# ooowedyn/InkLayer

Measured on AMD Instinct MI355X. Metric: sketches/sec end-to-end (GroundingDINO+SAM) at 1024x1024, higher is better.
Workload: dtype f16 (MFMA, f32 accumulate; f32 residual/norm/softmax; split-f16 = fp32-grade operands for patch-embed, neck, mask decoder)

## Files before the change

### include/inklayer_hip.h

```cpp
#ifndef INKLAYER_HIP_H
#define INKLAYER_HIP_H

#include <stdint.h>

#ifdef __cplusplus
extern "C" {
#endif

#define INK_ABI_VERSION 8
int ink_abi_version(void);

typedef struct InkGemm {
  const void* A;
  const void* W;
  const float* bias;
  const float* col_scale;
  const float* residual;
  const int32_t* row_map;
  void* C;
  int32_t M, N, K;
  int32_t lda, ldw, ldr, ldc;
  int32_t act;
  int32_t c_f16;
} InkGemm;
#define INK_ACT_NONE 0
#define INK_ACT_GELU 1
#define INK_ACT_RELU 2
int ink_gemm_f16(const InkGemm* p, void* stream);
int ink_gemm_set_variant(int32_t v);
int ink_gemm_query_variant(int32_t M, int32_t N, int32_t K);

int ink_layernorm_rows(const float* x, int64_t ldx, const float* gamma, const float* beta,
                       float eps, const int32_t* gather, int32_t rows_out, int32_t C,
                       void* out_f16, float* out_f32, int64_t ldo, int32_t act, int32_t split,
                       const float* add, int64_t ld_add, const int32_t* add_batch_rows, int32_t rows_per_batch,
                       void* stream);

int ink_add_cvt_f16(const float* a, const float* b, int64_t n_b, void* out_f16, int64_t n,
                    void* stream);
int ink_add_split_f16(const float* a, const float* b, int64_t n_b, void* out_f16, int64_t n, int32_t C,
                      void* stream);
int ink_add_f32(const float* a, const float* b, int64_t n_b, float* out, int64_t n, void* stream);

typedef struct InkAttn {
  const void* Q; const void* K; const void* V;
  void* O;
  int64_t ldq, ldk, ldv, ldo;
  int32_t n_batch, n_heads, n_q, n_k, head_dim;
  float scale;
  int32_t bias_mode;
  int32_t grid_w;
  const int32_t* q_batch_rows;
  const int32_t* kv_batch_rows;
  const float* rel_h; const float* rel_w;
  const void* rel_aug;
  const float* dense_bias; const float* dense_mask;
  int32_t n_mask; int32_t rel_f16;
  const int32_t* tok_rows;
  const void* pad_k; const void* pad_v;
} InkAttn;
int ink_flash_attn(const InkAttn* p, void* stream);

int ink_relpos_bias64_f16(const void* Q, int64_t ldq, const float* rel_pos_h, const float* rel_pos_w, int32_t n_batch,
                          int32_t n_heads, int32_t head_dim, float scale, void* out_h_f16, void* out_w_f16, void* stream);

int ink_relpos_bias(const void* Q, int64_t ldq, const float* rel_pos_h, const float* rel_pos_w,
                    int32_t S, int32_t n_batch, int32_t n_heads, int32_t head_dim, float scale,
                    const int32_t* tok_rows, float* out_h, float* out_w, void* out_aug_f16,
                    void* stream);

int ink_sam_patchify(const void* image_u8, int32_t h, int32_t w, int32_t L, int32_t P,
                     const float* mean3, const float* std3, int32_t chan_reverse, int32_t split,
                     void* out_f16, void* stream);

int ink_resize_bilinear_u8(const void* src_u8, int32_t h, int32_t w, void* dst_u8, int32_t oh, int32_t ow,
                           const int32_t* xbounds, const int32_t* xcoef, int32_t kx,
                           const int32_t* ybounds, const int32_t* ycoef, int32_t ky, void* tmp_u8,
                           void* stream);

int ink_im2col3x3_f16(const void* in_f16, int32_t B, int32_t H, int32_t W, int32_t C, void* out_f16,
                      void* stream);

int ink_sam_pe_encode(const float* coords01, const float* gauss, int32_t N, int32_t F,
                      const float* add, int32_t n_add, float* out, void* stream);

int ink_sam_prompt_tokens(const float* points, const int32_t* labels, int32_t n_pts, int32_t pad, const float* boxes,
                          const float* gauss, int32_t F, const float* point_emb, const float* not_a_point,
                          const float* out_tok, float input_size, int32_t P, float* out, void* stream);

int ink_sam_mask_embed(const float* mask, const float* emb, const int32_t* emb_rows, const float* params,
                       int32_t n_params, float eps, int32_t P, int32_t g, float* keys, void* split_f16, void* stream);

int ink_sam_mask_logits(const float* up, const float* hyper, int32_t n, int32_t g, int32_t C,
                        float* out, void* stream);

int ink_sam_postprocess(const float* low, int32_t n, int32_t S, int32_t L, int32_t in_h,
                        int32_t in_w, int32_t out_h, int32_t out_w, float thr, void* out_u8,
                        float* out_logits, void* stream);

int ink_ms_deform_attn_forward(const float* value, const int64_t* spatial_shapes_host,
                               const int64_t* level_start_index_host, const float* sampling_loc,
                               const float* attn_weight, int32_t B, int32_t S, int32_t M, int32_t C,
                               int32_t Q, int32_t L, int32_t P, int32_t im2col_step, float* out,
                               void* stream);

int ink_ms_deform_attn_forward_dev(const void* value, const int64_t* spatial_shapes,
                                   const int64_t* level_start_index, const void* sampling_loc,
                                   const void* attn_weight, int32_t dtype, int32_t B, int32_t S, int32_t M,
                                   int32_t C, int32_t Q, int32_t L, int32_t P, int32_t im2col_step,
                                   void* out, void* stream);
int ink_ms_deform_attn_backward_dev(const void* value, const int64_t* spatial_shapes,
                                    const int64_t* level_start_index, const void* sampling_loc,
                                    const void* attn_weight, const void* grad_output, int32_t dtype,
                                    int32_t B, int32_t S, int32_t M, int32_t C, int32_t Q, int32_t L,
                                    int32_t P, int32_t im2col_step, void* grad_value,
                                    void* grad_sampling_loc, void* grad_attn_weight, void* stream);

int ink_msda_fused(const void* value_f16, const float* proj, int64_t ldp, const float* ref,
                   int32_t ref_dim, int64_t ref_q_stride, int64_t ref_b_stride,
                   const int32_t* shapes_host, int32_t B, int32_t S, int32_t Q, void* out_f16,
                   void* stream);

int ink_swin_patchify(const void* image_u8, int32_t h, int32_t w, const float* mean3,
                      const float* std3, void* out_f16, void* stream);

int ink_layernorm_merge4(const float* x, int64_t ldx, const float* gamma, const float* beta, float eps,
                         const int32_t* gather4, int32_t rows, int32_t C, void* out_f16, void* stream);

int ink_groupnorm_nhwc(const float* x, int32_t B, int32_t T, int32_t C, int32_t G, const float* gamma,
                       const float* beta, float eps, float* stats_ws, float* out,
                       int64_t out_batch_stride, void* stream);

int ink_gather_rows(const float* x, int64_t ldx, int64_t x_batch_rows, const int32_t* idx,
                    int64_t idx_batch_stride, int32_t rows_per_batch, int32_t B, int32_t C,
                    void* out_f16, float* out_f32, void* stream);

int ink_biattn_fusion(const void* QV_f16, const void* KL_f16, int32_t B, int32_t S, int32_t T, int32_t E,
                      float scale, float* scores_ws, float* stats_ws, float* partial_ws, int32_t chunk,
                      void* out_v_f16, void* out_l_f16, void* stream);

int ink_attn_fewkeys(const void* Q, int64_t ldq, const void* K, int64_t ldk, const void* V, int64_t ldv,
                     int32_t B, int32_t n_q, int32_t n_k, int32_t n_heads, int32_t head_dim, float scale,
                     const uint8_t* blocked, const int32_t* q_batch_rows, const float* q_add, int32_t io_f32, void* O,
                     int64_t ldo, void* stream);

int ink_attn_fewq(const void* Q, int64_t ldq, const void* K, int64_t ldk, const void* V, int64_t ldv,
                  int32_t n_batch, int32_t n_q, int32_t n_k, int32_t n_heads, int32_t head_dim, float scale,
                  const int32_t* q_batch_rows, const int32_t* kv_batch_rows, const float* k_add, void* O, int64_t ldo,
                  void* stream);

int ink_biattn_colstats(const float* scores, int32_t B, int32_t S, int32_t HT, float* part_ws, float* stats, void* stream);

int ink_fusion_fold_workspace(int32_t B, int32_t S, int64_t* out_floats);
int ink_fusion_fold(float* v_f32, int32_t B, int32_t S, const float* lnv_g, const float* lnv_b, float eps,
                    const float* text_k_f32, const float* text_vl_f32, int64_t ld_text, int32_t T, const void* Wq_f16,
                    const float* bq, const void* Wvv_f16, const float* bvv, const void* Wo_f16, const float* bo,
                    const float* gamma_v, float scale, float* ws, void* out_l_f16, const float* pos, void* out16_pos,
                    void* out16, void* stream);

int ink_sam_upscale_pack(const void* ws_f16, void* blob_f16, void* stream);
int ink_sam_upscale_tail(const float* u0, int64_t ld_tok, int32_t n, int32_t g, const float* ln_g, const float* ln_b, float eps,
                         const void* blob_f16, const float* b3, const float* hyper, int32_t n_masks, float* low,
                         void* stream);

int ink_proj256_ln_pack(const void* ws_f16, void* blob_f16, void* stream);
int ink_proj256_ln(const float* a_f32, const void* blob_f16, const float* bias, const float* res_f32,
                   const int32_t* res_batch_rows, int32_t rows_per_batch, const float* ln_g, const float* ln_b, float eps,
                   int64_t rows, float* out_f32, void* out_split_f16, void* stream);

int ink_ffn256_pack_bytes(int32_t hid, int32_t with_pre, int64_t* out_bytes);
int ink_ffn256_pack(const void* w1_f16, const float* b1, const void* w2_f16, int32_t hid, const void* wpre_f16, void* blob,
                    void* stream);
int ink_ffn256_fused(const void* x_f16, int64_t ldx, const float* res_f32, const void* blob, const float* b2,
                     const float* ln_g, const float* ln_b, float eps, int32_t M, int32_t hid, const float* pre_bias,
                     const float* pre_ln_g, const float* pre_ln_b, float* out_f32, void* stream);

int ink_topk_rowmax(const float* logits, int32_t B, int32_t S, int32_t T, int32_t K, int32_t* out_idx,
                    float* out_val, void* cand_ws, void* stream);

int ink_sine_embed4(const float* ref, const float* dim_t, int32_t N, void* out_f16, void* stream);

int ink_box_refine(const float* delta, int64_t ldd, const float* ref, int32_t N, int32_t ref_is_logit,
                   float* out, void* stream);

int ink_mask_cleanup_workspace_ints(int32_t n, int32_t H, int32_t W, int32_t k, int64_t* out_ints);
int ink_mask_cleanup(const void* masks_u8, int32_t n, int32_t H, int32_t W, int32_t k, int32_t area_threshold,
                     double aspect_threshold, void* tmp_a_u8, void* tmp_b_u8, int32_t* workspace, void* out_u8,
                     void* stream);

int ink_mask_sketch_iou_counts(const void* masks_u8, const void* sketch_rgb_u8, int32_t n, int32_t H, int32_t W,
                               void* bits_ws_u64, int32_t* counts, void* stream);

int ink_sam_amg_stats(const float* low, int32_t n, const int32_t* index, int32_t m, const int32_t* m_dev, int32_t S,
                      int32_t L, int32_t in_h, int32_t in_w, int32_t crop_h, int32_t crop_w, double thr, double offset,
                      int32_t x0, int32_t y0, int32_t orig_h, int32_t orig_w, int32_t* table, void* planes_u64,
                      float* out_logits, void* stream);

int ink_mask_rle_counts(const void* planes_u64, const int32_t* select, int32_t k, int32_t H, int32_t W,
                        int32_t* n_counts, void* stream);
int ink_mask_rle_write(const void* planes_u64, const int32_t* select, int32_t k, int32_t H, int32_t W,
                       const int32_t* offsets, int32_t* counts, void* stream);

int ink_mask_small_regions_workspace_ints(int32_t k, int32_t H, int32_t W, int64_t* out_ints);
int ink_mask_small_regions(const void* planes_u64, int32_t k, int32_t H, int32_t W, int32_t min_area, int32_t holes,
                           void* tmp_planes_u64, int32_t* workspace, void* out_planes_u64, int32_t* changed, void* stream);

int ink_box_nms(const float* boxes, const float* scores, int32_t n, float iou_threshold, void* workspace_u64,
                int32_t* keep, int32_t* n_keep, void* stream);

int ink_refine_sketch_planes(const void* rgb_u8, int32_t H, int32_t W, void* planes4_u64, int32_t* max_ws, void* stream);

int ink_bitplane_pack(const void* img_u8, int32_t n, int32_t H, int32_t W, int32_t thresh, void* planes_u64, void* stream);

int ink_refine_depth_samples(const void* mask_planes, int32_t n, const float* depth, const int32_t* pts_yx, int32_t P,
                             int32_t H, int32_t W, float* vals, void* inside_u8, void* stream);

int ink_refine_pair_tables(const void* mask_planes, const void* sketch_planes4, int32_t n, int32_t H, int32_t W,
                           const int32_t* rect, void* dil_ws_planes, int32_t* pair, int32_t* per_mask,
                           int32_t* sketch_area, void* stream);

int ink_refine_composite(const void* mask_planes, const int32_t* order, int32_t n_ranks, int32_t H, int32_t W,
                         void* label_u8, int32_t* hist256, void* stream);

int ink_refine_relabel_clean(const void* label_u8, const void* map256_u8, int32_t H, int32_t W, void* out_label_u8,
                             void* stream);

int ink_refine_grow_workspace(int32_t H, int32_t W, int64_t* plane_words, int64_t* cc_ints);
int ink_refine_grow(const void* label_u8, const void* sketch_planes4, int32_t H, int32_t W, void* planes_ws,
                    int32_t* cc_ws, int32_t* flags256, void* out_label_u8, int32_t* bbox256x4, int32_t* unl_yx,
                    int32_t unl_cap, int32_t* unl_count, void* stream);

int ink_refine_query_dists(const void* label_u8, const int32_t* q_yx, const void* cand256_bits, int32_t Q, int32_t H,
                           int32_t W, int32_t* d2_Qx256, void* stream);

int ink_refine_finalize(void* label_u8, const int32_t* assign_yxl, int32_t A, const void* sketch_planes4, int32_t H,
                        int32_t W, void* planes_ws3, void* extra_plane, int32_t* extra_count, void* stream);

int ink_host_sparse_sample(const uint8_t* rgb_u8, int32_t H, int32_t W, int32_t* out_yx, int32_t cap, int32_t* count);
int ink_host_assign_unlabeled(const int32_t* q_yx, int32_t Q, const int32_t* boxes, int32_t nb, const int32_t* box2mask,
                              const int32_t* d2, const uint8_t* nonempty, int32_t n_masks, int32_t* out_label);

int ink_depth_patchify(const void* image_u8, int32_t H, int32_t W, int32_t nh, int32_t nw, int32_t P, int32_t KP,
                       const double* mean3, const double* std3, int32_t chan_reverse, void* out_f16, void* stream);

int ink_resize_bilinear_ac_nhwc(const float* in, int32_t B, int32_t h, int32_t w, int32_t C, int32_t H, int32_t W,
                                float* out_f32, void* out_f16, void* stream);

int ink_im2col3x3_ex_f16(const void* in_f16, int32_t B, int32_t H, int32_t W, int32_t C, int32_t stride, int32_t relu,
                         void* out_f16, void* stream);

int ink_layers_otsu_planes(const void* gray_u8, int32_t n, int32_t H, int32_t W, int32_t invert, int32_t* hist,
                           int32_t* thresh, void* out_planes, void* stream);

int ink_layers_dilate(const void* planes, int32_t n, int32_t H, int32_t W, int32_t kernel_size, int32_t iterations,
                      void* tmp_planes, void* out_planes, void* stream);

int ink_layers_border_band(const void* planes, int32_t n, int32_t H, int32_t W, int32_t band, int32_t* flags,
                           void* stream);

int ink_layers_components_workspace_ints(int32_t n, int32_t H, int32_t W, int64_t* out_ints);
int ink_layers_components(const void* planes, int32_t n, int32_t H, int32_t W, int32_t mode, void* tmp_planes3,
                          int32_t* workspace, void* out_planes, void* stream);

int ink_layers_chamfer_workspace_ints(int32_t n, int32_t H, int32_t W, int64_t* out_ints);
int ink_layers_chamfer(const void* mask_planes, const void* stroke_planes, int32_t n, int32_t H, int32_t W,
                       int32_t safety_margin, int32_t full, int32_t* dist, int32_t* workspace, int32_t* min_out,
                       int32_t* shrink_out, void* out_planes, void* stream);

int ink_layers_mask_tables(const void* masks_u8, int32_t n, int32_t H, int32_t W, int32_t* bbox, int32_t* overlap,
                           void* stream);

int ink_layers_assemble(const void* sketch_rgb_u8, const void* masks_u8, const void* bg_planes, const int32_t* bbox,
                        const int32_t* overlap, int32_t n, int32_t H, int32_t W, void* sketch_layers_u8,
                        void* edit_masks_u8, void* debug_u8, void* stream);

int ink_layers_composite(const void* inpainted_rgb_u8, const void* sketch_layer_u8, int32_t H, int32_t W,
                         void* out_rgb_u8, void* stream);

int ink_layers_gray(const void* rgb_u8, int32_t n, int32_t H, int32_t W, void* gray_u8, void* stream);

int ink_layers_rgba(const void* gray_u8, const void* bg_planes, int32_t n, int32_t H, int32_t W, void* rgba_u8,
                    void* stream);


int ink_inp_contrast(const void* rgb_u8, int32_t H, int32_t W, float factor, void* sum_u64, void* out_rgb_u8,
                     void* stream);

int ink_inp_bilateral(const void* rgb_u8, int32_t H, int32_t W, const float* tables, void* out_rgb_u8, void* stream);

int ink_inp_mask_prepare(const void* mask_u8, int32_t H, int32_t W, int32_t dilate_iterations, int32_t blur,
                         void* tmp2_u8, void* out_u8, void* stream);

int ink_inp_resize_u8(const void* src_u8, int32_t h, int32_t w, int32_t channels, void* dst_u8, int32_t oh, int32_t ow,
                      const int32_t* xbounds, const int32_t* xcoef, int32_t kx, const int32_t* ybounds,
                      const int32_t* ycoef, int32_t ky, void* tmp_u8, void* stream);

int ink_inp_condition(const void* rgb_u8, const void* mask_u8, int32_t H, int32_t W, float* out_f32, void* stream);
// ... 19 lines not shown
```

### inklayer_amd/_lib.py

```python
from __future__ import annotations

import ctypes as C
import os
from pathlib import Path

_LIB_PATH = Path(__file__).resolve().parent / "lib" / "libinklayer_hip.so"
_lib = None

c_void_p, c_int, c_i64, c_float = C.c_void_p, C.c_int32, C.c_int64, C.c_float


class InkGemm(C.Structure):
    _fields_ = [
        ("A", c_void_p), ("W", c_void_p), ("bias", c_void_p), ("col_scale", c_void_p),
        ("residual", c_void_p), ("row_map", c_void_p), ("C", c_void_p),
        ("M", c_int), ("N", c_int), ("K", c_int),
        ("lda", c_int), ("ldw", c_int), ("ldr", c_int), ("ldc", c_int),
        ("act", c_int), ("c_f16", c_int),
    ]


class InkAttn(C.Structure):
    _fields_ = [
        ("Q", c_void_p), ("K", c_void_p), ("V", c_void_p), ("O", c_void_p),
        ("ldq", c_i64), ("ldk", c_i64), ("ldv", c_i64), ("ldo", c_i64),
        ("n_batch", c_int), ("n_heads", c_int), ("n_q", c_int), ("n_k", c_int),
        ("head_dim", c_int), ("scale", c_float), ("bias_mode", c_int), ("grid_w", c_int),
        ("q_batch_rows", c_void_p), ("kv_batch_rows", c_void_p),
        ("rel_h", c_void_p), ("rel_w", c_void_p), ("rel_aug", c_void_p),
        ("dense_bias", c_void_p), ("dense_mask", c_void_p), ("n_mask", c_int), ("rel_f16", c_int),
        ("tok_rows", c_void_p), ("pad_k", c_void_p), ("pad_v", c_void_p),
    ]


SIGNATURES = {
    "ink_abi_version": [],
    "ink_gemm_f16": [C.POINTER(InkGemm), c_void_p],
    "ink_gemm_set_variant": [c_int],
    "ink_gemm_query_variant": [c_int, c_int, c_int],
    "ink_layernorm_rows": [c_void_p, c_i64, c_void_p, c_void_p, c_float, c_void_p, c_int, c_int,
                           c_void_p, c_void_p, c_i64, c_int, c_int, c_void_p, c_i64, c_void_p, c_int, c_void_p],
    "ink_add_split_f16": [c_void_p, c_void_p, c_i64, c_void_p, c_i64, c_int, c_void_p],
    "ink_add_cvt_f16": [c_void_p, c_void_p, c_i64, c_void_p, c_i64, c_void_p],
    "ink_add_f32": [c_void_p, c_void_p, c_i64, c_void_p, c_i64, c_void_p],
    "ink_flash_attn": [C.POINTER(InkAttn), c_void_p],
    "ink_sam_patchify": [c_void_p, c_int, c_int, c_int, c_int, C.POINTER(c_float), C.POINTER(c_float),
                         c_int, c_int, c_void_p, c_void_p],
    "ink_im2col3x3_f16": [c_void_p, c_int, c_int, c_int, c_int, c_void_p, c_void_p],
    "ink_resize_bilinear_u8": [c_void_p, c_int, c_int, c_void_p, c_int, c_int, c_void_p, c_void_p, c_int,
                               c_void_p, c_void_p, c_int, c_void_p, c_void_p],
    "ink_sam_pe_encode": [c_void_p, c_void_p, c_int, c_int, c_void_p, c_int, c_void_p, c_void_p],
    "ink_sam_mask_logits": [c_void_p, c_void_p, c_int, c_int, c_int, c_void_p, c_void_p],
    "ink_sam_prompt_tokens": [c_void_p, c_void_p, c_int, c_int, c_void_p, c_void_p, c_int, c_void_p, c_void_p,
                              c_void_p, c_float, c_int, c_void_p, c_void_p],
    "ink_sam_mask_embed": [c_void_p, c_void_p, c_void_p, c_void_p, c_int, c_float, c_int, c_int, c_void_p, c_void_p,
                           c_void_p],
    "ink_sam_postprocess": [c_void_p, c_int, c_int, c_int, c_int, c_int, c_int, c_int, c_float,
                            c_void_p, c_void_p, c_void_p],
    "ink_sam_amg_stats": [c_void_p, c_int, c_void_p, c_int, c_void_p, c_int, c_int, c_int, c_int, c_int, c_int, C.c_double,
                          C.c_double, c_int, c_int, c_int, c_int, c_void_p, c_void_p, c_void_p, c_void_p],
    "ink_mask_rle_counts": [c_void_p, c_void_p, c_int, c_int, c_int, c_void_p, c_void_p],
    "ink_mask_rle_write": [c_void_p, c_void_p, c_int, c_int, c_int, c_void_p, c_void_p, c_void_p],
    "ink_mask_small_regions_workspace_ints": [c_int, c_int, c_int, C.POINTER(c_i64)],
    "ink_mask_small_regions": [c_void_p, c_int, c_int, c_int, c_int, c_int, c_void_p, c_void_p, c_void_p, c_void_p,
                               c_void_p],
    "ink_box_nms": [c_void_p, c_void_p, c_int, c_float, c_void_p, c_void_p, c_void_p, c_void_p],
    "ink_ms_deform_attn_forward": [c_void_p, C.POINTER(c_i64), C.POINTER(c_i64), c_void_p, c_void_p, c_int,
                                   c_int, c_int, c_int, c_int, c_int, c_int, c_int, c_void_p, c_void_p],
    "ink_ms_deform_attn_forward_dev": [c_void_p, c_void_p, c_void_p, c_void_p, c_void_p, c_int, c_int, c_int, c_int,
                                       c_int, c_int, c_int, c_int, c_int, c_void_p, c_void_p],
    "ink_ms_deform_attn_backward_dev": [c_void_p, c_void_p, c_void_p, c_void_p, c_void_p, c_void_p, c_int, c_int, c_int,
                                        c_int, c_int, c_int, c_int, c_int, c_int, c_void_p, c_void_p, c_void_p,
                                        c_void_p],
    "ink_msda_fused": [c_void_p, c_void_p, c_i64, c_void_p, c_int, c_i64, c_i64, C.POINTER(c_int), c_int,
                       c_int, c_int, c_void_p, c_void_p],
    "ink_swin_patchify": [c_void_p, c_int, c_int, C.POINTER(c_float), C.POINTER(c_float), c_void_p, c_void_p],
    "ink_layernorm_merge4": [c_void_p, c_i64, c_void_p, c_void_p, c_float, c_void_p, c_int, c_int, c_void_p,
                             c_void_p],
    "ink_groupnorm_nhwc": [c_void_p, c_int, c_int, c_int, c_int, c_void_p, c_void_p, c_float, c_void_p,
                           c_void_p, c_i64, c_void_p],
    "ink_gather_rows": [c_void_p, c_i64, c_i64, c_void_p, c_i64, c_int, c_int, c_int, c_void_p, c_void_p,
                        c_void_p],
    "ink_biattn_fusion": [c_void_p, c_void_p, c_int, c_int, c_int, c_int, c_float, c_void_p, c_void_p,
                          c_void_p, c_int, c_void_p, c_void_p, c_void_p],
    "ink_biattn_colstats": [c_void_p, c_int, c_int, c_int, c_void_p, c_void_p, c_void_p],
    "ink_fusion_fold_workspace": [c_int, c_int, C.POINTER(c_i64)],
    "ink_relpos_bias64_f16": [c_void_p, c_i64, c_void_p, c_void_p, c_int, c_int, c_int, c_float, c_void_p, c_void_p, c_void_p],
    "ink_proj256_ln_pack": [c_void_p, c_void_p, c_void_p],
    "ink_proj256_ln": [c_void_p, c_void_p, c_void_p, c_void_p, c_void_p, c_int, c_void_p, c_void_p, c_float, c_i64, c_void_p,
                       c_void_p, c_void_p],
    "ink_sam_upscale_pack": [c_void_p, c_void_p, c_void_p],
    "ink_sam_upscale_tail": [c_void_p, c_i64, c_int, c_int, c_void_p, c_void_p, c_float, c_void_p, c_void_p, c_void_p,
                             c_int, c_void_p, c_void_p],
    "ink_ffn256_pack_bytes": [c_int, c_int, C.POINTER(c_i64)],
    "ink_ffn256_pack": [c_void_p, c_void_p, c_void_p, c_int, c_void_p, c_void_p, c_void_p],
    "ink_ffn256_fused": [c_void_p, c_i64, c_void_p, c_void_p, c_void_p, c_void_p, c_void_p, c_float, c_int, c_int,
                         c_void_p, c_void_p, c_void_p, c_void_p, c_void_p],
    "ink_fusion_fold": [c_void_p, c_int, c_int, c_void_p, c_void_p, c_float, c_void_p, c_void_p, c_i64, c_int, c_void_p,
                        c_void_p, c_void_p, c_void_p, c_void_p, c_void_p, c_void_p, c_float, c_void_p, c_void_p, c_void_p,
                        c_void_p, c_void_p, c_void_p],
    "ink_attn_fewkeys": [c_void_p, c_i64, c_void_p, c_i64, c_void_p, c_i64, c_int, c_int, c_int, c_int, c_int,
                         c_float, c_void_p, c_void_p, c_void_p, c_int, c_void_p, c_i64, c_void_p],
    "ink_attn_fewq": [c_void_p, c_i64, c_void_p, c_i64, c_void_p, c_i64, c_int, c_int, c_int, c_int, c_int,
                      c_float, c_void_p, c_void_p, c_void_p, c_void_p, c_i64, c_void_p],
    "ink_topk_rowmax": [c_void_p, c_int, c_int, c_int, c_int, c_void_p, c_void_p, c_void_p, c_void_p],
    "ink_sine_embed4": [c_void_p, c_void_p, c_int, c_void_p, c_void_p],
    "ink_box_refine": [c_void_p, c_i64, c_void_p, c_int, c_int, c_void_p, c_void_p],
    "ink_mask_cleanup_workspace_ints": [c_int, c_int, c_int, c_int, C.POINTER(c_i64)],
    "ink_mask_cleanup": [c_void_p, c_int, c_int, c_int, c_int, c_int, C.c_double, c_void_p, c_void_p, c_void_p,
                         c_void_p, c_void_p],
    "ink_mask_sketch_iou_counts": [c_void_p, c_void_p, c_int, c_int, c_int, c_void_p, c_void_p, c_void_p],
    "ink_refine_sketch_planes": [c_void_p, c_int, c_int, c_void_p, c_void_p, c_void_p],
    "ink_bitplane_pack": [c_void_p, c_int, c_int, c_int, c_int, c_void_p, c_void_p],
    "ink_refine_depth_samples": [c_void_p, c_int, c_void_p, c_void_p, c_int, c_int, c_int, c_void_p, c_void_p, c_void_p],
    "ink_refine_pair_tables": [c_void_p, c_void_p, c_int, c_int, c_int, c_void_p, c_void_p, c_void_p, c_void_p,
                               c_void_p, c_void_p],
    "ink_refine_composite": [c_void_p, c_void_p, c_int, c_int, c_int, c_void_p, c_void_p, c_void_p],
    "ink_refine_relabel_clean": [c_void_p, c_void_p, c_int, c_int, c_void_p, c_void_p],
    "ink_refine_grow_workspace": [c_int, c_int, C.POINTER(c_i64), C.POINTER(c_i64)],
    "ink_refine_grow": [c_void_p, c_void_p, c_int, c_int, c_void_p, c_void_p, c_void_p, c_void_p, c_void_p, c_void_p,
                        c_int, c_void_p, c_void_p],
    "ink_refine_query_dists": [c_void_p, c_void_p, c_void_p, c_int, c_int, c_int, c_void_p, c_void_p],
    "ink_refine_finalize": [c_void_p, c_void_p, c_int, c_void_p, c_int, c_int, c_void_p, c_void_p, c_void_p, c_void_p],
    "ink_host_sparse_sample": [c_void_p, c_int, c_int, c_void_p, c_int, c_void_p],
    "ink_host_assign_unlabeled": [c_void_p, c_int, c_void_p, c_int, c_void_p, c_void_p, c_void_p, c_int, c_void_p],
    "ink_depth_patchify": [c_void_p, c_int, c_int, c_int, c_int, c_int, c_int, C.POINTER(C.c_double), C.POINTER(C.c_double),
                           c_int, c_void_p, c_void_p],
    "ink_resize_bilinear_ac_nhwc": [c_void_p, c_int, c_int, c_int, c_int, c_int, c_int, c_void_p, c_void_p, c_void_p],
    "ink_im2col3x3_ex_f16": [c_void_p, c_int, c_int, c_int, c_int, c_int, c_int, c_void_p, c_void_p],
    "ink_layers_otsu_planes": [c_void_p, c_int, c_int, c_int, c_int, c_void_p, c_void_p, c_void_p, c_void_p],
    "ink_layers_dilate": [c_void_p, c_int, c_int, c_int, c_int, c_int, c_void_p, c_void_p, c_void_p],
    "ink_layers_border_band": [c_void_p, c_int, c_int, c_int, c_int, c_void_p, c_void_p],
    "ink_layers_components_workspace_ints": [c_int, c_int, c_int, C.POINTER(c_i64)],
    "ink_layers_components": [c_void_p, c_int, c_int, c_int, c_int, c_void_p, c_void_p, c_void_p, c_void_p],
    "ink_layers_chamfer_workspace_ints": [c_int, c_int, c_int, C.POINTER(c_i64)],
    "ink_layers_chamfer": [c_void_p, c_void_p, c_int, c_int, c_int, c_int, c_int, c_void_p, c_void_p, c_void_p, c_void_p,
                           c_void_p, c_void_p],
    "ink_layers_mask_tables": [c_void_p, c_int, c_int, c_int, c_void_p, c_void_p, c_void_p],
    "ink_layers_assemble": [c_void_p, c_void_p, c_void_p, c_void_p, c_void_p, c_int, c_int, c_int, c_void_p, c_void_p,
                            c_void_p, c_void_p],
    "ink_layers_composite": [c_void_p, c_void_p, c_int, c_int, c_void_p, c_void_p],
    "ink_layers_gray": [c_void_p, c_int, c_int, c_int, c_void_p, c_void_p],
    "ink_layers_rgba": [c_void_p, c_void_p, c_int, c_int, c_int, c_void_p, c_void_p],
    "ink_inp_contrast": [c_void_p, c_int, c_int, c_float, c_void_p, c_void_p, c_void_p],
    "ink_inp_bilateral": [c_void_p, c_int, c_int, c_void_p, c_void_p, c_void_p],
    "ink_inp_mask_prepare": [c_void_p, c_int, c_int, c_int, c_int, c_void_p, c_void_p, c_void_p],
    "ink_inp_resize_u8": [c_void_p, c_int, c_int, c_int, c_void_p, c_int, c_int, c_void_p, c_void_p, c_int,
                          c_void_p, c_void_p, c_int, c_void_p, c_void_p],
    "ink_inp_condition": [c_void_p, c_void_p, c_int, c_int, c_void_p, c_void_p],
    "ink_inp_cleanup": [c_void_p, c_int, c_int, c_void_p, c_void_p, c_void_p, c_void_p, c_void_p],
    "ink_inp_soft_blend": [c_void_p, c_void_p, c_void_p, c_int, c_int, c_void_p, c_void_p, c_void_p, c_void_p],
    "ink_inp_luma": [c_void_p, c_int, c_int, c_int, c_void_p, c_void_p],
    "ink_inp_unsharp": [c_void_p, c_int, c_int, c_int, C.c_uint32, C.c_uint32, c_int, c_int, c_void_p, c_void_p, c_void_p],
    "ink_inp_rgba_cut": [c_void_p, c_void_p, c_int, c_int, c_void_p, c_void_p],
    "ink_relpos_bias": [c_void_p, c_i64, c_void_p, c_void_p, c_int, c_int, c_int, c_int, c_float,
                        c_void_p, c_void_p, c_void_p, c_void_p, c_void_p],
}


class InkLayerHipError(RuntimeError):
    pass


def lib_path() -> Path:
    return Path(os.environ.get("INKLAYER_HIP_LIB", _LIB_PATH))


def lib() -> C.CDLL:
    global _lib
    if _lib is None:
        p = lib_path()
        if not p.exists():
            raise InkLayerHipError(
                f"{p} not found: build it with `python -m inklayer_amd.build` "
                "(there is no CPU/eager fallback for the InkLayer hot path)")
        try:
            import torch
        except ImportError:
            pass
        l = C.CDLL(str(p))
        for name, argtypes in SIGNATURES.items():
            fn = getattr(l, name)
            fn.argtypes = argtypes
            fn.restype = C.c_int
        _lib = l
    return _lib


def check(rc: int, what: str) -> None:
    if rc != 0:
        raise InkLayerHipError(f"{what} failed: " + {1: "bad argument", 2: "HIP launch error"}.get(rc, str(rc)))
```

### inklayer_amd/csrc/attn_few.hip

```cpp
#include "common.h"
#include "../../include/inklayer_hip.h"

namespace {

__device__ __forceinline__ void load8(const f16* p, float* d) {
  const f16x8 v = *(const f16x8*)p;
#pragma unroll
  for (int j = 0; j < 8; ++j) d[j] = (float)v[j];
}
__device__ __forceinline__ void load8(const float* p, float* d) {
  const f32x4 a = *(const f32x4*)p, b = *(const f32x4*)(p + 4);
#pragma unroll
  for (int j = 0; j < 4; ++j) { d[j] = a[j]; d[4 + j] = b[j]; }
}
__device__ __forceinline__ void store8(f16* p, const float* d) {
  f16x8 v;
#pragma unroll
  for (int j = 0; j < 8; ++j) v[j] = (f16)d[j];
  *(f16x8*)p = v;
}
__device__ __forceinline__ void store8(float* p, const float* d) {
  *(f32x4*)p = (f32x4){d[0], d[1], d[2], d[3]};
  *(f32x4*)(p + 4) = (f32x4){d[4], d[5], d[6], d[7]};
}

template <int HD, typename T>
__global__ __launch_bounds__(256) void attn_fewkeys_kernel(const T* __restrict__ Q, int64_t ldq,
                                                           const T* __restrict__ K, int64_t ldk,
                                                           const T* __restrict__ V, int64_t ldv, int B,
                                                           int n_q, int n_k, int n_heads, float scale,
                                                           const uint8_t* __restrict__ blocked,
                                                           const int32_t* __restrict__ q_rows,
                                                           const float* __restrict__ q_add,
                                                           T* __restrict__ O, int64_t ldo) {
  const int64_t gid = (int64_t)blockIdx.x * 256 + threadIdx.x;
  if (gid >= (int64_t)B * n_q * n_heads) return;
  const int h = (int)(gid % n_heads);
  const int64_t bq = gid / n_heads;
  const int b = (int)(bq / n_q), q = (int)(bq % n_q);
  float qv[HD];
  const T* qp = Q + (q_rows ? (int64_t)q_rows[b] + q : bq) * ldq + h * HD;
#pragma unroll
  for (int i = 0; i < HD / 8; ++i) load8(qp + 8 * i, qv + 8 * i);
  if (q_add) {
    const float* ap = q_add + ((int64_t)q * n_heads + h) * HD;
#pragma unroll
    for (int i = 0; i < HD; ++i) qv[i] += ap[i];
  }
  float sc[16];
  float mx = -3.0e38f;
  for (int t = 0; t < n_k; ++t) {
    const T* kp = K + ((int64_t)b * n_k + t) * ldk + h * HD;
    float d = 0.f;
#pragma unroll
    for (int i = 0; i < HD / 8; ++i) {
      float kv[8];
      load8(kp + 8 * i, kv);
#pragma unroll
      for (int j = 0; j < 8; ++j) d = fmaf(qv[8 * i + j], kv[j], d);
    }
    d *= scale;
    if (blocked && blocked[q * n_k + t]) d = -3.0e38f;
    sc[t] = d;
    mx = fmaxf(mx, d);
  }
  float sum = 0.f;
  for (int t = 0; t < n_k; ++t) { sc[t] = sc[t] <= -1.0e38f ? 0.f : expf(sc[t] - mx); sum += sc[t]; }
  const float inv = 1.f / sum;
  float acc[HD];
#pragma unroll
  for (int i = 0; i < HD; ++i) acc[i] = 0.f;
  for (int t = 0; t < n_k; ++t) {
    const T* vp = V + ((int64_t)b * n_k + t) * ldv + h * HD;
    const float pw = sc[t] * inv;
#pragma unroll
    for (int i = 0; i < HD / 8; ++i) {
      float vv[8];
      load8(vp + 8 * i, vv);
#pragma unroll
      for (int j = 0; j < 8; ++j) acc[8 * i + j] = fmaf(pw, vv[j], acc[8 * i + j]);
    }
  }
  T* op = O + bq * ldo + h * HD;
#pragma unroll
  for (int i = 0; i < HD / 8; ++i) store8(op + 8 * i, acc + 8 * i);
}


template <int NK>
__global__ __launch_bounds__(256) void attn_fewkeys16_f32_kernel(const float* __restrict__ Q, int64_t ldq,
                                                                 const float* __restrict__ K, int64_t ldk,
                                                                 const float* __restrict__ V, int64_t ldv, int B,
                                                                 int n_q, int n_heads, float scale,
                                                                 const int32_t* __restrict__ q_rows,
                                                                 const float* __restrict__ q_add,
                                                                 float* __restrict__ O, int64_t ldo) {
  const int64_t gid = (int64_t)blockIdx.x * 256 + threadIdx.x;
  if (gid >= (int64_t)B * n_q * n_heads * 4) return;
  const int part = (int)(gid & 3);
  const int h = (int)((gid >> 2) % n_heads);
  const int64_t bq = (gid >> 2) / n_heads;
  const int b = (int)(bq / n_q), q = (int)(bq % n_q);
  const int col = h * 16 + 4 * part;
  f32x4 qv = *(const f32x4*)(Q + (q_rows ? (int64_t)q_rows[b] + q : bq) * ldq + col);
  if (q_add) qv += *(const f32x4*)(q_add + (int64_t)q * n_heads * 16 + col);
  qv *= scale * 1.44269504088896340736f;
  const float* kp = K + (int64_t)b * NK * ldk + col;
  const float* vp = V + (int64_t)b * NK * ldv + col;
  f32x4 kv[NK], vv[NK];
#pragma unroll
  for (int t = 0; t < NK; ++t) {
    kv[t] = *(const f32x4*)(kp + (int64_t)t * ldk);
    vv[t] = *(const f32x4*)(vp + (int64_t)t * ldv);
  }
  float sc[NK];
  float mx = -3.0e38f;
#pragma unroll
  for (int t = 0; t < NK; ++t) {
    float d = (qv[0] * kv[t][0] + qv[1] * kv[t][1]) + (qv[2] * kv[t][2] + qv[3] * kv[t][3]);
    d += __builtin_bit_cast(float, __builtin_amdgcn_update_dpp(0, __builtin_bit_cast(int, d), 0xB1, 0xF, 0xF, false));
    d += __builtin_bit_cast(float, __builtin_amdgcn_update_dpp(0, __builtin_bit_cast(int, d), 0x4E, 0xF, 0xF, false));
    sc[t] = d;
    mx = fmaxf(mx, d);
  }
  float sum = 0.f;
#pragma unroll
  for (int t = 0; t < NK; ++t) { sc[t] = __builtin_amdgcn_exp2f(sc[t] - mx); sum += sc[t]; }
  const float inv = 1.f / sum;
  f32x4 acc = {0.f, 0.f, 0.f, 0.f};
#pragma unroll
  for (int t = 0; t < NK; ++t) acc += (sc[t] * inv) * vv[t];
  *(f32x4*)(O + bq * ldo + col) = acc;
}

template <int QW>
__global__ __launch_bounds__(512) void attn_fewq16_kernel(const float* __restrict__ Q, int64_t ldq,
                                                          const float* __restrict__ K, int64_t ldk,
                                                          const float* __restrict__ V, int64_t ldv, int n_q,
                                                          int n_k, int n_heads, float scale,
                                                          const int32_t* __restrict__ q_rows,
                                                          const int32_t* __restrict__ kv_rows,
                                                          const float* __restrict__ k_add,
                                                          float* __restrict__ O, int64_t ldo) {
  constexpr int KSPLIT = 2, HD = 16, HB = 4, TK = 64;
  constexpr int ROWE = HB * HD;
  constexpr int CH = 4, NCH = ROWE / CH;
  constexpr int NU = TK * NCH / 256;
  constexpr bool Q_IN_LDS = QW > 2;
  extern __shared__ __attribute__((aligned(16))) char fewq_smem[];
  const int grp = threadIdx.x >> 8;
  float* sk = (float*)fewq_smem + grp * 2 * TK * ROWE;
  float* sv = sk + TK * ROWE;
  const int hgroups = n_heads / HB;
  const int b = blockIdx.x / hgroups, h0 = (blockIdx.x % hgroups) * HB;
  const int tid = threadIdx.x & 255, lane = tid & 63, wave = tid >> 6;
  const int per = ((n_k + KSPLIT - 1) / KSPLIT + TK - 1) / TK * TK;
  const int k_lo = grp * per, k_hi = min(n_k, k_lo + per);
  const int kl = lane >> 2, hl = lane & 3;
  const int64_t q0 = q_rows ? (int64_t)q_rows[b] : (int64_t)b * n_q;
  const int64_t k0 = kv_rows ? (int64_t)kv_rows[b] : (int64_t)b * n_k;
  float* sq = (float*)fewq_smem + KSPLIT * 2 * TK * ROWE;
  float qr[QW][HD];
  if (!Q_IN_LDS || (grp == 0 && kl == 0)) {
    const float sc2 = scale * 1.44269504088896340736f;
#pragma unroll
    for (int j = 0; j < QW; ++j) {
      const int qi = QW * wave + j;
      const float* pq = Q + (q0 + (qi < n_q ? qi : 0)) * ldq + (h0 + hl) * HD;
      load8(pq, qr[j]);
      load8(pq + 8, qr[j] + 8);
#pragma unroll
      for (int e = 0; e < HD; ++e) qr[j][e] *= sc2;
      if constexpr (Q_IN_LDS) {
        store8(sq + (qi * HB + hl) * HD, qr[j]);
        store8(sq + (qi * HB + hl) * HD + 8, qr[j] + 8);
      }
    }
  }
  float m[QW], l[QW], acc[QW][HD];
#pragma unroll
  for (int j = 0; j < QW; ++j) {
    m[j] = -3.0e38f;
    l[j] = 0.f;
#pragma unroll
    for (int i = 0; i < HD; ++i) acc[j][i] = 0.f;
  }
  f32x4 rk[NU], rv[NU];
  auto fetch = [&](int t0) {
#pragma unroll
    for (int u = 0; u < NU; ++u) {
      const int c = tid + 256 * u, row = c / NCH, col = c % NCH;
      rk[u] = rv[u] = (f32x4){0.f, 0.f, 0.f, 0.f};
      if (t0 + row < k_hi) {
        rk[u] = *(const f32x4*)(K + (k0 + t0 + row) * ldk + h0 * HD + col * CH);
        rv[u] = *(const f32x4*)(V + (k0 + t0 + row) * ldv + h0 * HD + col * CH);
        if (k_add) rk[u] += *(const f32x4*)(k_add + (int64_t)(t0 + row) * n_heads * HD + h0 * HD + col * CH);
      }
    }
  };
  fetch(k_lo);
  for (int t0 = k_lo; t0 < k_lo + per; t0 += TK) {
    __syncthreads();
#pragma unroll
    for (int u = 0; u < NU; ++u) {
      const int c = tid + 256 * u, row = c / NCH, col = c % NCH;
      *(f32x4*)(sk + row * ROWE + col * CH) = rk[u];
      *(f32x4*)(sv + row * ROWE + col * CH) = rv[u];
    }
    __syncthreads();
    if (t0 + TK < k_hi) fetch(t0 + TK);
    float d[QW][TK / 16];
#pragma unroll
    for (int kk = 0; kk < TK / 16; ++kk) {
      const int key = kk * 16 + kl;
      float kf[HD];
      load8(sk + key * ROWE + hl * HD, kf);
      load8(sk + key * ROWE + hl * HD + 8, kf + 8);
      const bool in = t0 + key < k_hi;
#pragma unroll
      for (int j = 0; j < QW; ++j) {
        float qf[HD];
        if constexpr (Q_IN_LDS) {
          load8(sq + ((QW * wave + j) * HB + hl) * HD, qf);
          load8(sq + ((QW * wave + j) * HB + hl) * HD + 8, qf + 8);
        } else {
#pragma unroll
          for (int e = 0; e < HD; ++e) qf[e] = qr[j][e];
        }
        float a0 = 0.f;
#pragma unroll
        for (int e = 0; e < 8; ++e) {
          a0 = fmaf(qf[e], kf[e], a0);
          a0 = fmaf(qf[8 + e], kf[8 + e], a0);
        }
        d[j][kk] = in ? a0 : -3.0e38f;
      }
    }
    float n[QW];
#pragma unroll
    for (int j = 0; j < QW; ++j) {
      n[j] = m[j];
#pragma unroll
      for (int kk = 0; kk < TK / 16; ++kk) n[j] = fmaxf(n[j], d[j][kk]);
      const float sj = __builtin_amdgcn_exp2f(m[j] - n[j]);
      l[j] *= sj;
#pragma unroll
      for (int e = 0; e < HD; ++e) acc[j][e] *= sj;
      m[j] = n[j];
    }
#pragma unroll
    for (int kk = 0; kk < TK / 16; ++kk) {
      const int key = kk * 16 + kl;
      float vf[HD];
      load8(sv + key * ROWE + hl * HD, vf);
      load8(sv + key * ROWE + hl * HD + 8, vf + 8);
      const bool in = t0 + key < k_hi;
#pragma unroll
      for (int j = 0; j < QW; ++j) {
        const float pj = in ? __builtin_amdgcn_exp2f(d[j][kk] - n[j]) : 0.f;
        l[j] += pj;
#pragma unroll
        for (int e = 0; e < HD; ++e) acc[j][e] = fmaf(pj, vf[e], acc[j][e]);
      }
    }
  }
#pragma unroll
  for (int j = 0; j < QW; ++j) {
#pragma unroll
    for (int o = 4; o < 64; o <<= 1) {
      const float mo = __shfl_xor(m[j], o, 64), lo = __shfl_xor(l[j], o, 64);
      const float mn = fmaxf(m[j], mo);
      const float a = __builtin_amdgcn_exp2f(m[j] - mn), bsc = __builtin_amdgcn_exp2f(mo - mn);
      l[j] = l[j] * a + lo * bsc;
#pragma unroll
      for (int i = 0; i < HD; ++i) acc[j][i] = acc[j][i] * a + __shfl_xor(acc[j][i], o, 64) * bsc;
      m[j] = mn;
    }
  }
  __syncthreads();
  float* st = (float*)fewq_smem;
  if (grp > 0 && kl == 0) {
#pragma unroll
    for (int j = 0; j < QW; ++j) {
      float* ps = st + ((((grp - 1) * 4 + wave) * QW + j) * 4 + hl) * 18;
      ps[0] = m[j];
      ps[1] = l[j];
#pragma unroll
      for (int i = 0; i < HD; ++i) ps[2 + i] = acc[j][i];
    }
  }
  __syncthreads();
  if (grp > 0) return;
  if (kl == 0) {
#pragma unroll
    for (int g2 = 1; g2 < KSPLIT; ++g2)
#pragma unroll
      for (int j = 0; j < QW; ++j) {
        const float* ps = st + ((((g2 - 1) * 4 + wave) * QW + j) * 4 + hl) * 18;
        const float mo = ps[0], mn = fmaxf(m[j], mo);
        const float a = __builtin_amdgcn_exp2f(m[j] - mn), bsc = __builtin_amdgcn_exp2f(mo - mn);
        l[j] = l[j] * a + ps[1] * bsc;
#pragma unroll
        for (int i = 0; i < HD; ++i) acc[j][i] = acc[j][i] * a + ps[2 + i] * bsc;
        m[j] = mn;
      }
#pragma unroll
    for (int j = 0; j < QW; ++j) {
      const int qi = QW * wave + j;
      if (qi < n_q) {
        const float inv = 1.f / l[j];
#pragma unroll
        for (int i = 0; i < HD; ++i) acc[j][i] *= inv;
        float* op = O + ((int64_t)b * n_q + qi) * ldo + (h0 + hl) * HD;
        store8(op, acc[j]);
        store8(op + 8, acc[j] + 8);
      }
    }
  }
}

}

extern "C" int ink_attn_fewkeys(const void* Q, int64_t ldq, const void* K, int64_t ldk, const void* V,
                                int64_t ldv, int32_t B, int32_t n_q, int32_t n_k, int32_t n_heads,
                                int32_t head_dim, float scale, const uint8_t* blocked,
                                const int32_t* q_batch_rows, const float* q_add, int32_t io_f32, void* O,
                                int64_t ldo, void* stream) {
  INK_CHECK_ARG(Q && K && V && O && B > 0 && n_q > 0 && n_k > 0 && n_k <= 16 && n_heads > 0);
  INK_CHECK_ARG(ldq % 8 == 0 && ldk % 8 == 0 && ldv % 8 == 0 && ldo % 8 == 0);
  INK_CHECK_ARG(io_f32 == 0 || io_f32 == 1);
  INK_CHECK_ARG((((uintptr_t)Q | (uintptr_t)K | (uintptr_t)V | (uintptr_t)O) & 15) == 0);
  INK_CHECK_ARG(!q_add || (((uintptr_t)q_add & 15) == 0));
  const int64_t total = (int64_t)B * n_q * n_heads;
  const dim3 grid((unsigned)((total + 255) / 256)), block(256);
  hipStream_t s = (hipStream_t)stream;
#define INK_FEWKEYS(HD, T)                                                                                     \
  hipLaunchKernelGGL((attn_fewkeys_kernel<HD, T>), grid, block, 0, s, (const T*)Q, ldq, (const T*)K, ldk,      \
                     (const T*)V, ldv, B, n_q, n_k, n_heads, scale, blocked, q_batch_rows, q_add, (T*)O, ldo)
  if (head_dim == 32 && !io_f32) INK_FEWKEYS(32, f16);
  else if (head_dim == 64 && !io_f32) INK_FEWKEYS(64, f16);
  else if (!io_f32) return INK_ERR_ARG;
  else if (head_dim == 32) INK_FEWKEYS(32, float);
  else if (head_dim == 16 && !blocked && n_k >= 7) {
    const dim3 g4((unsigned)((total * 4 + 255) / 256));
#define INK_FEWKEYS16(NK)                                                                                        \
  case NK:                                                                                                      \
    hipLaunchKernelGGL(attn_fewkeys16_f32_kernel<NK>, g4, block, 0, s, (const float*)Q, ldq, (const float*)K, ldk, \
                       (const float*)V, ldv, B, n_q, n_heads, scale, q_batch_rows, q_add, (float*)O, ldo);         \
    break
    switch (n_k) {
      INK_FEWKEYS16(7); INK_FEWKEYS16(8); INK_FEWKEYS16(9); INK_FEWKEYS16(10); INK_FEWKEYS16(11);
      INK_FEWKEYS16(12); INK_FEWKEYS16(13); INK_FEWKEYS16(14); INK_FEWKEYS16(15); INK_FEWKEYS16(16);
      default: return INK_ERR_ARG;
    }
#undef INK_FEWKEYS16
  } else if (head_dim == 16) INK_FEWKEYS(16, float);
  else return INK_ERR_ARG;
#undef INK_FEWKEYS
  return ink_launch_status();
}

extern "C" int ink_attn_fewq(const void* Q, int64_t ldq, const void* K, int64_t ldk, const void* V, int64_t ldv,
                             int32_t n_batch, int32_t n_q, int32_t n_k, int32_t n_heads, int32_t head_dim,
                             float scale, const int32_t* q_batch_rows, const int32_t* kv_batch_rows,
                             const float* k_add, void* O, int64_t ldo, void* stream) {
  INK_CHECK_ARG(Q && K && V && O && n_batch > 0 && n_q > 0 && n_q <= 16 && n_k > 0 && n_heads > 0);
  INK_CHECK_ARG(head_dim == 16 && n_heads % 4 == 0);
  INK_CHECK_ARG(ldq % 8 == 0 && ldk % 8 == 0 && ldv % 8 == 0 && ldo % 8 == 0);
  INK_CHECK_ARG((((uintptr_t)Q | (uintptr_t)K | (uintptr_t)V | (uintptr_t)O) & 15) == 0);
  INK_CHECK_ARG(!k_add || ((uintptr_t)k_add & 15) == 0);
  constexpr int lds2 = 2 * 2 * 64 * 64 * 4, lds4 = lds2 + 16 * 64 * 4;
  static bool attr = ((void)hipFuncSetAttribute((const void*)attn_fewq16_kernel<2>,
                                                hipFuncAttributeMaxDynamicSharedMemorySize, lds2),
                      (void)hipFuncSetAttribute((const void*)attn_fewq16_kernel<4>,
                                                hipFuncAttributeMaxDynamicSharedMemorySize, lds4), true);
  (void)attr;
  const bool wide = n_q > 8;
  hipLaunchKernelGGL(wide ? attn_fewq16_kernel<4> : attn_fewq16_kernel<2>, dim3(n_batch * (n_heads / 4)), dim3(512),
                     wide ? lds4 : lds2, (hipStream_t)stream, (const float*)Q, ldq, (const float*)K, ldk,
                     (const float*)V, ldv, n_q, n_k, n_heads, scale, q_batch_rows, kv_batch_rows, k_add, (float*)O, ldo);
  return ink_launch_status();
}
```

### inklayer_amd/csrc/common.h

```cpp
#pragma once
#include <hip/hip_runtime.h>
#include <stdint.h>

typedef _Float16 f16;
typedef _Float16 f16x2 __attribute__((ext_vector_type(2)));
typedef _Float16 f16x4 __attribute__((ext_vector_type(4)));
typedef _Float16 f16x8 __attribute__((ext_vector_type(8)));
typedef float f32x2 __attribute__((ext_vector_type(2)));
typedef float f32x4 __attribute__((ext_vector_type(4)));
typedef float f32x16 __attribute__((ext_vector_type(16)));
typedef short s16x4 __attribute__((ext_vector_type(4)));

#define INK_OK 0
#define INK_ERR_ARG 1
#define INK_ERR_LAUNCH 2

#define INK_CHECK_ARG(cond)            \
  do {                                 \
    if (!(cond)) return INK_ERR_ARG;   \
  } while (0)

static inline int ink_launch_status() {
  hipError_t e = hipGetLastError();
  return e == hipSuccess ? INK_OK : INK_ERR_LAUNCH;
}

__device__ __forceinline__ float wave_sum(float v) {
#pragma unroll
  for (int o = 32; o > 0; o >>= 1) v += __shfl_xor(v, o, 64);
  return v;
}
__device__ __forceinline__ float wave_max(float v) {
#pragma unroll
  for (int o = 32; o > 0; o >>= 1) v = fmaxf(v, __shfl_xor(v, o, 64));
  return v;
}

__device__ __forceinline__ float gelu_erf(float x) {
  const float u = fabsf(x) * 0.84932180028801904272f;
  const float t = __builtin_amdgcn_rcpf(fmaf(0.27273748087922250f, u, 1.0f));
  float pl = fmaf(1.061405429f, t, -1.453152027f);
  pl = fmaf(pl, t, 1.421413741f);
  pl = fmaf(pl, t, -0.284496736f);
  pl = fmaf(pl, t, 0.254829592f);
  const float e = pl * t * __builtin_amdgcn_exp2f(-(u * u));
  return fmaf(-0.5f * fabsf(x), e, fmaxf(x, 0.0f));
}

__device__ __forceinline__ int xcd_remap(int bid, int nwg) {
  const int q = nwg >> 3, r = nwg & 7, x = bid & 7;
  return (x < r ? x * (q + 1) : r * (q + 1) + (x - r) * q) + (bid >> 3);
}
```

### inklayer_amd/csrc/gemm.hip

```cpp
#include <stdlib.h>

#include "common.h"
#include "../../include/inklayer_hip.h"

namespace {

template <int BK> struct Swz;
template <> struct Swz<64> {
  static __device__ __forceinline__ int f(int row) { return row & 7; }
};
template <> struct Swz<32> {
  static __device__ __forceinline__ int f(int row) { return (-(row >> 2)) & 3; }
};

typedef __attribute__((address_space(1))) const void* gptr_t;
typedef __attribute__((address_space(3))) void* lptr_t;

__device__ __forceinline__ bool residual_preloaded(const InkGemm& p) {
  return p.residual && p.act == INK_ACT_NONE && !p.col_scale;
}

template <int TM>
__device__ __forceinline__ void wave_rows(int (&rows)[TM], const InkGemm& p, int mw, int lane) {
#pragma unroll
  for (int ti = 0; ti < TM; ++ti) {
    const int m = mw + ti * 16 + (lane & 15);
    int r = -1;
    if (m < p.M) r = p.row_map ? p.row_map[m] : m;
    rows[ti] = r;
  }
}

template <int TM, int TN>
__device__ __forceinline__ void init_wave_tile(f32x4 (&acc)[TM][TN], const InkGemm& p, const int (&rows)[TM], int nw,
                                               int lane) {
  const int fq = lane >> 4;
  const bool pre = residual_preloaded(p);
#pragma unroll
  for (int ti = 0; ti < TM; ++ti) {
    const int r = pre ? rows[ti] : -1;
    const float* rp = p.residual + (size_t)max(r, 0) * p.ldr + nw + fq * 4;
#pragma unroll
    for (int j = 0; j < TN; ++j) {
      acc[ti][j] = (f32x4){0.f, 0.f, 0.f, 0.f};
      if (r >= 0 && nw + j * 16 + fq * 4 < p.N) acc[ti][j] = *(const f32x4*)(rp + j * 16);
    }
  }
}

template <int TM, int TN>
__device__ __forceinline__ void add_bias_wave_tile(f32x4 (&acc)[TM][TN], const InkGemm& p, int nw, int lane) {
  const int fq = lane >> 4;
#pragma unroll
  for (int j = 0; j < TN; ++j) {
    const int n = nw + j * 16 + fq * 4;
    f32x4 bv = (f32x4){0.f, 0.f, 0.f, 0.f};
    if (p.bias && n < p.N) bv = *(const f32x4*)(p.bias + n);
#pragma unroll
    for (int ti = 0; ti < TM; ++ti) acc[ti][j] += bv;
  }
}

template <int TM, int TN, int OUT, int MODE = -1>
__device__ __forceinline__ void store_wave_tile(f32x4 (&acc)[TM][TN], const InkGemm& p, char* er,
                                                const int (&rows)[TM], int nw, int lane) {
  constexpr bool F16O = OUT == 1;
  constexpr int WNC = TN * 16, EP = WNC * 4 + 16;
  constexpr int ES = OUT == 0 ? 4 : 8;
  constexpr int CPRW = WNC / ES;
  constexpr int NIT = (16 * CPRW + 63) / 64;
  const int fr = lane & 15, fq = lane >> 4;
  const bool wide16 = OUT != 0 && (p.ldc % 8 == 0);
  const bool res_late = MODE < 0 && p.residual && !residual_preloaded(p);
  const int act = MODE < 0 ? p.act : MODE;
  const bool scaled = MODE < 0 && p.col_scale != nullptr;
  int row_of[NIT], n_of[NIT];
#pragma unroll
  for (int it = 0; it < NIT; ++it) {
    const int c = it * 64 + lane;
    row_of[it] = c < 16 * CPRW ? c / CPRW : 16;
    n_of[it] = nw + (c % CPRW) * ES;
  }

  add_bias_wave_tile<TM, TN>(acc, p, nw, lane);

#pragma unroll
  for (int ti = 0; ti < TM; ++ti) {
#pragma unroll
    for (int j = 0; j < TN; ++j) {
      f32x4 v = acc[ti][j];
      if (act == INK_ACT_GELU) {
#pragma unroll
        for (int r = 0; r < 4; ++r) v[r] = gelu_erf(v[r]);
      } else if (act == INK_ACT_RELU) {
#pragma unroll
        for (int r = 0; r < 4; ++r) v[r] = fmaxf(v[r], 0.f);
      }
      if (scaled) {
        const int n = nw + j * 16 + fq * 4;
        if (n < p.N) v *= *(const f32x4*)(p.col_scale + n);
      }
      if (F16O) {
        *(f16x4*)(er + fr * EP + (j * 16 + fq * 4) * 2) = (f16x4){(f16)v[0], (f16)v[1], (f16)v[2], (f16)v[3]};
      } else {
        *(f32x4*)(er + fr * EP + (j * 16 + fq * 4) * 4) = v;
      }
    }
#pragma unroll
    for (int it = 0; it < NIT; ++it) {
      int r = __builtin_amdgcn_ds_bpermute((row_of[it] & 15) << 2, rows[ti]);
      if (row_of[it] >= 16 || n_of[it] >= p.N) r = -1;
      if (r >= 0) {
        const int c_n = n_of[it];
        const char* src = er + row_of[it] * EP + (c_n - nw) * (F16O ? 2 : 4);
        if (F16O) {
          f16x8 d = *(const f16x8*)src;
          f16* dst = (f16*)p.C + (size_t)r * p.ldc + c_n;
          if (res_late) {
            const float* rp = p.residual + (size_t)r * p.ldr + c_n;
#pragma unroll
            for (int e = 0; e < 8; ++e)
              if (c_n + e < p.N) d[e] = (f16)((float)d[e] + rp[e]);
          }
          if (wide16 && c_n + 8 <= p.N) {
            *(f16x8*)dst = d;
          } else {
            *(f16x4*)dst = (f16x4){d[0], d[1], d[2], d[3]};
            if (c_n + 8 <= p.N) *(f16x4*)(dst + 4) = (f16x4){d[4], d[5], d[6], d[7]};
          }
        } else {
          f32x4 d = *(const f32x4*)src;
          if (res_late) d += *(const f32x4*)(p.residual + (size_t)r * p.ldr + c_n);
          *(f32x4*)((float*)p.C + (size_t)r * p.ldc + c_n) = d;
        }
      }
    }
  }
}

__device__ __forceinline__ void tile_of(int id, int ntm, int ntn, int group_m, int& mt, int& nt) {
  if (group_m > 1) {
    const int per = group_m * ntn;
    const int first = (id / per) * group_m;
    const int gsz = min(ntm - first, group_m);
    mt = first + (id % per) % gsz;
    nt = (id % per) / gsz;
  } else {
    mt = id / ntn;
    nt = id % ntn;
  }
}

constexpr int NS = 2;
template <int BM, int BN, int BK, int WM, int WN>
__global__ __launch_bounds__(WM * WN * 64) void gemm_f16_nt(InkGemm p, int group_m) {
  constexpr int NT = WM * WN * 64;
  constexpr int CPR = BK / 8;
  constexpr int ROWB = BK * 2;
  constexpr int TILE_A = BM * ROWB, TILE_W = BN * ROWB;
  constexpr int STAGE = TILE_A + TILE_W;
  constexpr int IT_A = (BM * CPR) / NT, IT_W = (BN * CPR) / NT;
  constexpr int TM = BM / WM / 16, TN = BN / WN / 16;
  static_assert((BM * CPR) % NT == 0 && (BN * CPR) % NT == 0, "tile/threads mismatch");
  extern __shared__ __attribute__((aligned(16))) char smem[];

  const int tid = threadIdx.x;
  const int lane = tid & 63;
  const int wave = tid >> 6;
  const int wm = wave / WN, wn = wave % WN;

  const int ntn = (p.N + BN - 1) / BN;
  const int ntm = (p.M + BM - 1) / BM;
  int mt, nt;
  tile_of(xcd_remap(blockIdx.x, ntm * ntn), ntm, ntn, group_m, mt, nt);
  const int m0 = mt * BM;
  const int n0 = nt * BN;

  const f16* __restrict__ A = (const f16*)p.A;
  const f16* __restrict__ W = (const f16*)p.W;

  const f16* srcA[IT_A];
  const f16* srcW[IT_W];
#pragma unroll
  for (int it = 0; it < IT_A; ++it) {
    const int pch = it * NT + tid;
    const int row = pch / CPR;
    const int lch = (pch % CPR) ^ Swz<BK>::f(row);
    srcA[it] = A + (size_t)min(m0 + row, p.M - 1) * p.lda + lch * 8;
  }
#pragma unroll
  for (int it = 0; it < IT_W; ++it) {
    const int pch = it * NT + tid;
    const int row = pch / CPR;
    const int lch = (pch % CPR) ^ Swz<BK>::f(row);
    srcW[it] = W + (size_t)min(n0 + row, p.N - 1) * p.ldw + lch * 8;
  }

  auto stage = [&](int buf, int kt) {
    char* base = smem + buf * STAGE;
#pragma unroll
    for (int it = 0; it < IT_A; ++it)
      __builtin_amdgcn_global_load_lds((gptr_t)(srcA[it] + kt * BK), (lptr_t)(base + (it * NT + wave * 64) * 16), 16, 0, 0);
#pragma unroll
    for (int it = 0; it < IT_W; ++it)
      __builtin_amdgcn_global_load_lds((gptr_t)(srcW[it] + kt * BK), (lptr_t)(base + TILE_A + (it * NT + wave * 64) * 16), 16, 0, 0);
  };

  int rows[TM];
  wave_rows<TM>(rows, p, m0 + wm * (BM / WM), lane);
  f32x4 acc[TM][TN];

  const int fr = lane & 15, fq = lane >> 4;
  const int offA = (wm * (BM / WM) + fr) * ROWB;
  const int offW = (wn * (BN / WN) + fr) * ROWB;
  const int swz = Swz<BK>::f(fr);

  const int nk = p.K / BK;
  auto compute = [&](int cur) {
    const char* bA = smem + cur * STAGE;
    const char* bW = bA + TILE_A;
#pragma unroll
    for (int kk = 0; kk < BK / 32; ++kk) {
      constexpr int AG = TM > 4 ? 4 : TM;
      f16x8 a[AG], w[TN];
      const int co = ((kk * 4 + fq) ^ swz) << 4;
#pragma unroll
      for (int j = 0; j < TN; ++j) w[j] = *(const f16x8*)(bW + offW + j * 16 * ROWB + co);
#pragma unroll
      for (int i0 = 0; i0 < TM; i0 += AG) {
#pragma unroll
        for (int i = 0; i < AG; ++i) a[i] = *(const f16x8*)(bA + offA + (i0 + i) * 16 * ROWB + co);
#pragma unroll
        for (int i = 0; i < AG; ++i)
#pragma unroll
          for (int j = 0; j < TN; ++j)
            acc[i0 + i][j] = __builtin_amdgcn_mfma_f32_16x16x32_f16(w[j], a[i], acc[i0 + i][j], 0, 0, 0);
      }
    }
  };

  stage(0, 0);
  init_wave_tile<TM, TN>(acc, p, rows, n0 + wn * (BN / WN), lane);
  for (int kt = 0; kt < nk; ++kt) {
    asm volatile("s_waitcnt vmcnt(0)" ::: "memory");
    __syncthreads();
    if (kt + 1 < nk) stage((kt + 1) & 1, kt + 1);
    compute(kt & 1);
  }

  constexpr int WNC = BN / WN;
  constexpr int EP = WNC * 4 + 16;
  static_assert(WM * WN * 16 * EP <= NS * STAGE, "epilogue patch must fit in the staging LDS");
  __syncthreads();
  char* er = smem + wave * (16 * EP);
  if (p.c_f16 == 1) {
    store_wave_tile<TM, TN, 1>(acc, p, er, rows, n0 + wn * WNC, lane);
  } else {
    store_wave_tile<TM, TN, 0>(acc, p, er, rows, n0 + wn * WNC, lane);
  }
}

constexpr int PP_RING = 4, PP_TN = 5;
__global__ __launch_bounds__(512) void gemm_f16_nt_pp(InkGemm p, int group_m) {
  constexpr int RING = PP_RING, TN = PP_TN;
  constexpr int BM = 256, BN = 64 * TN, BK = 32, NT = 512;
  constexpr int CPR = BK / 8, ROWB = BK * 2;
  constexpr int TILE_A = BM * ROWB, TILE_W = BN * ROWB, GRAN = TILE_A + TILE_W;
  constexpr int IT_A = (BM * CPR) / NT, IT_W = (BN * CPR) / NT;
  constexpr bool W_TAIL = (BN * CPR) % NT != 0;
  static_assert(!W_TAIL || (BN * CPR) % NT == NT / 2, "tail is exactly the first four waves");
  constexpr int LOADS = IT_A + IT_W;
  constexpr int TM = 8, WNC = 16 * TN;
  constexpr int AHEAD = RING - 2;
  constexpr int AG = 4;
  constexpr int EP = WNC * 4 + 16;
  static_assert(8 * 16 * EP <= RING * GRAN, "patch fits");
  extern __shared__ __attribute__((aligned(16))) char smem[];
  const int tid = threadIdx.x, lane = tid & 63;
  const int wave = __builtin_amdgcn_readfirstlane(tid >> 6);
  const int grp = wave >> 2, wn = wave & 3;
  const int fr = lane & 15, fq = lane >> 4;

  const int ntn = (p.N + BN - 1) / BN, ntm = (p.M + BM - 1) / BM;
  int mt, nt;
  tile_of(xcd_remap(blockIdx.x, ntm * ntn), ntm, ntn, group_m, mt, nt);
  const int m0 = mt * BM, n0 = nt * BN;
  const int G = p.K / BK;
  const f16* __restrict__ A = (const f16*)p.A;
  const f16* __restrict__ W = (const f16*)p.W;
  const f16* srcA[IT_A];
  const f16* srcW[IT_W + (W_TAIL ? 1 : 0)];
#pragma unroll
  for (int it = 0; it < IT_A; ++it) {
    const int pch = it * NT + tid, row = pch / CPR, lch = (pch % CPR) ^ Swz<BK>::f(row);
    srcA[it] = A + (size_t)min(m0 + row, p.M - 1) * p.lda + lch * 8;
  }
#pragma unroll
  for (int it = 0; it < IT_W + (W_TAIL ? 1 : 0); ++it) {
    const int pch = it * NT + tid, row = min(pch / CPR, BN - 1), lch = (pch % CPR) ^ Swz<BK>::f(row);
    srcW[it] = W + (size_t)min(n0 + row, p.N - 1) * p.ldw + lch * 8;
  }
  auto dma = [&](int g, int slot) {
    char* base = smem + slot * GRAN;
#pragma unroll
    for (int it = 0; it < IT_A; ++it)
      __builtin_amdgcn_global_load_lds((gptr_t)(srcA[it] + g * BK), (lptr_t)(base + (it * NT + wave * 64) * 16), 16, 0, 0);
#pragma unroll
    for (int it = 0; it < IT_W; ++it)
      __builtin_amdgcn_global_load_lds((gptr_t)(srcW[it] + g * BK), (lptr_t)(base + TILE_A + (it * NT + wave * 64) * 16), 16, 0, 0);
    if (W_TAIL && grp == 0)
      __builtin_amdgcn_global_load_lds((gptr_t)(srcW[IT_W] + g * BK), (lptr_t)(base + TILE_A + (IT_W * NT + wave * 64) * 16), 16, 0, 0);
  };
  auto wait_ahead = [&]() {
    if (W_TAIL && grp == 0) {
      asm volatile("s_waitcnt vmcnt(%0)" ::"n"((AHEAD - 1) * (LOADS + 1)) : "memory");
    } else {
      asm volatile("s_waitcnt vmcnt(%0)" ::"n"((AHEAD - 1) * LOADS) : "memory");
    }
  };
  auto slot_end = [&]() {
    __builtin_amdgcn_sched_barrier(0);
    __builtin_amdgcn_s_barrier();
    __builtin_amdgcn_sched_barrier(0);
  };

  int rows[TM];
  wave_rows<TM>(rows, p, m0 + grp * 128, lane);
#pragma unroll
  for (int g = 0; g < AHEAD; ++g) dma(g, g);
  f32x4 acc[TM][TN];
  init_wave_tile<TM, TN>(acc, p, rows, n0 + wn * WNC, lane);
  if (residual_preloaded(p)) {
    asm volatile("s_waitcnt vmcnt(0)" ::: "memory");
  } else {
    wait_ahead();
  }
  slot_end();
  if (grp == 1) slot_end();

  const int offA = (grp * 128 + fr) * ROWB;
  const int offW = (wn * WNC + fr) * ROWB;
  const int co = (fq ^ Swz<BK>::f(fr)) << 4;
  f16x8 a[AG], w[TN];
  int cslot = 0, islot = AHEAD % RING;
  auto iter = [&](int g) __attribute__((always_inline)) {
    const char* bA = smem + cslot * GRAN;
    const char* bW = bA + TILE_A;
#pragma unroll
    for (int i = 0; i < AG; ++i) a[i] = *(const f16x8*)(bA + offA + i * 16 * ROWB + co);
#pragma unroll
    for (int j = 0; j < TN; ++j) w[j] = *(const f16x8*)(bW + offW + j * 16 * ROWB + co);
    if (g + AHEAD < G) {
      dma(g + AHEAD, islot);
      wait_ahead();
    } else {
      asm volatile("s_waitcnt vmcnt(0)" ::: "memory");
    }
    slot_end();
    asm volatile("s_waitcnt lgkmcnt(0)" ::: "memory");
    __builtin_amdgcn_sched_barrier(0);
    __builtin_amdgcn_s_setprio(1);
#pragma unroll
    for (int i0 = 0; i0 < TM; i0 += AG) {
#pragma unroll
      for (int i = 0; i < AG; ++i) {
#pragma unroll
        for (int j = 0; j < TN; ++j)
          acc[i0 + i][j] = __builtin_amdgcn_mfma_f32_16x16x32_f16(w[j], a[i], acc[i0 + i][j], 0, 0, 0);
        if (i0 + AG < TM) {
          a[i] = *(const f16x8*)(bA + offA + (i0 + AG + i) * 16 * ROWB + co);
          __builtin_amdgcn_sched_barrier(0);
        }
      }
    }
    __builtin_amdgcn_s_setprio(0);
    slot_end();
    cslot = (cslot + 1 == RING) ? 0 : cslot + 1;
    islot = (islot + 1 == RING) ? 0 : islot + 1;
  };
  for (int g = 0; g < G; ++g) iter(g);
  if (grp == 0) slot_end();

  char* er = smem + wave * (16 * EP);
  const bool plain = !p.col_scale && !(p.residual && !residual_preloaded(p));
  if (p.c_f16) {
    if (plain && p.act == INK_ACT_GELU) {
      store_wave_tile<TM, TN, 1, INK_ACT_GELU>(acc, p, er, rows, n0 + wn * WNC, lane);
    } else if (plain && p.act == INK_ACT_NONE) {
      store_wave_tile<TM, TN, 1, INK_ACT_NONE>(acc, p, er, rows, n0 + wn * WNC, lane);
    } else {
      store_wave_tile<TM, TN, 1>(acc, p, er, rows, n0 + wn * WNC, lane);
    }
  } else {
    if (plain && p.act == INK_ACT_NONE) {
      store_wave_tile<TM, TN, 0, INK_ACT_NONE>(acc, p, er, rows, n0 + wn * WNC, lane);
    } else {
      store_wave_tile<TM, TN, 0>(acc, p, er, rows, n0 + wn * WNC, lane);
    }
  }
}

static int launch_gemm_pp(const InkGemm& p, hipStream_t s, int group_m) {
  if (p.K / 32 < PP_RING) return INK_ERR_ARG;
  constexpr int BN = 64 * PP_TN;
  constexpr int lds = PP_RING * (256 + BN) * 32 * 2;
  static_assert(lds <= 160 * 1024, "LDS budget");
  static bool attr = ((void)hipFuncSetAttribute((const void*)gemm_f16_nt_pp,
                                                hipFuncAttributeMaxDynamicSharedMemorySize, lds), true);
  (void)attr;
  const int ntiles = ((p.M + 255) / 256) * ((p.N + BN - 1) / BN);
  hipLaunchKernelGGL(gemm_f16_nt_pp, dim3(ntiles), dim3(512), lds, s, p, group_m);
  return ink_launch_status();
}

template <int BM, int BN, int BK, int WM, int WN>
static int launch_gemm(const InkGemm& p, hipStream_t s, int group_m = 1) {
  constexpr int lds = NS * (BM + BN) * BK * 2;
  static_assert(lds <= 160 * 1024, "LDS budget");
  static bool attr = ((void)hipFuncSetAttribute((const void*)gemm_f16_nt<BM, BN, BK, WM, WN>,
                                                hipFuncAttributeMaxDynamicSharedMemorySize, lds), true);
  (void)attr;
  const int ntm = (p.M + BM - 1) / BM, ntn = (p.N + BN - 1) / BN;
  hipLaunchKernelGGL((gemm_f16_nt<BM, BN, BK, WM, WN>), dim3(ntm * ntn), dim3(WM * WN * 64), lds, s, p, group_m);
  return ink_launch_status();
}

}

static int g_variant = -1;
extern "C" int ink_gemm_query_variant(int32_t M, int32_t N, int32_t K) {
  if (K % 64 != 0) return 32;
  if (N % 320 == 0 && K >= 128 && (long)((M + 255) / 256) * (N / 320) >= 384) return 45;
  const long tiles256 = (long)((M + 255) / 256) * ((N + 255) / 256);
  const bool n_fits = (N % 256 == 0) || N >= 1024;
  return (tiles256 >= 200 && n_fits) ? 10 : 0;
}
extern "C" int ink_abi_version(void) { return INK_ABI_VERSION; }
extern "C" int ink_gemm_set_variant(int32_t v) {
  INK_CHECK_ARG(v == -1 || v == 0 || v == 10 || v == 45);
  g_variant = v;
  return INK_OK;
}

extern "C" int ink_gemm_f16(const InkGemm* pp, void* stream) {
  INK_CHECK_ARG(pp != nullptr);
  const InkGemm& p = *pp;
  INK_CHECK_ARG(p.A && p.W && p.C);
  INK_CHECK_ARG(p.M > 0 && p.N > 0 && p.K > 0);
  INK_CHECK_ARG(p.K % 32 == 0 && p.N % 4 == 0);
  INK_CHECK_ARG(p.lda % 8 == 0 && p.ldw % 8 == 0 && p.lda >= p.K && p.ldw >= p.K);
  INK_CHECK_ARG(p.ldc % 4 == 0 && p.ldc >= p.N);
  INK_CHECK_ARG(!p.residual || (p.ldr % 4 == 0 && p.ldr >= p.N));
  INK_CHECK_ARG(((uintptr_t)p.A & 15) == 0 && ((uintptr_t)p.W & 15) == 0);
  INK_CHECK_ARG(((uintptr_t)p.C & 15) == 0);
  INK_CHECK_ARG(p.act >= 0 && p.act <= 2);
  INK_CHECK_ARG(p.c_f16 == 0 || p.c_f16 == 1);
  hipStream_t s = (hipStream_t)stream;
  if (p.K % 64 != 0) return launch_gemm<128, 128, 32, 2, 2>(p, s);
  int v = g_variant;
  if (v < 0) v = ink_gemm_query_variant(p.M, p.N, p.K);
  switch (v) {
    case 10: return launch_gemm<256, 256, 64, 4, 4>(p, s, 4);
    case 45: return launch_gemm_pp(p, s, 4);
    default: return launch_gemm<128, 128, 64, 2, 2>(p, s);
  }
}
```

### inklayer_amd/csrc/norm.hip

```cpp
#include "common.h"
#include "../../include/inklayer_hip.h"

namespace {

__device__ __forceinline__ void split_store(f16* o, int C, const f32x4& y) {
  f16x4 hi, lo, hs;
#pragma unroll
  for (int e = 0; e < 4; ++e) {
    hi[e] = (f16)y[e];
    lo[e] = (f16)((y[e] - (float)hi[e]) * 64.0f);
    hs[e] = (f16)((float)hi[e] * 0.015625f);
  }
  *(f16x4*)o = hi;
  *(f16x4*)(o + C) = lo;
  *(f16x4*)(o + 2 * C) = hs;
}

template <int NV>
__global__ __launch_bounds__(256) void layernorm_rows_kernel(
    const float* __restrict__ x, int64_t ldx, const float* __restrict__ gamma,
    const float* __restrict__ beta, float eps, const int32_t* __restrict__ gather, int rows_out,
    int C, f16* __restrict__ out_h, float* __restrict__ out_f, int64_t ldo, int act, int split,
    const float* __restrict__ add, int64_t ld_add, const int32_t* __restrict__ add_batch_rows, int rows_per_batch) {
  const int lane = threadIdx.x & 63;
  const int row = blockIdx.x * 4 + (threadIdx.x >> 6);
  if (row >= rows_out) return;
  const int nv = C >> 2;
  const int64_t ldf = split ? ldo / 3 : ldo;
  const int src = gather ? gather[row] : row;
  if (src < 0) {
    for (int v = lane; v < nv; v += 64) {
      if (out_h && split) split_store(out_h + row * ldo + v * 4, C, (f32x4){0.f, 0.f, 0.f, 0.f});
      else if (out_h) *(f16x4*)(out_h + row * ldo + v * 4) = (f16x4){0, 0, 0, 0};
      if (out_f) *(f32x4*)(out_f + row * ldf + v * 4) = (f32x4){0.f, 0.f, 0.f, 0.f};
    }
    return;
  }
  const float* xr = x + (int64_t)src * ldx;
  const float* ar = nullptr;
  if (add) {
    const int b = row / rows_per_batch, i = row - b * rows_per_batch;
    ar = add + ((int64_t)(add_batch_rows ? add_batch_rows[b] : b * rows_per_batch) + i) * ld_add;
  }
  f32x4 r[NV];
  float s = 0.f;
#pragma unroll
  for (int j = 0; j < NV; ++j) {
    const int v = lane + 64 * j;
    r[j] = v < nv ? *(const f32x4*)(xr + v * 4) : (f32x4){0.f, 0.f, 0.f, 0.f};
    if (ar && v < nv) r[j] += *(const f32x4*)(ar + v * 4);
    s += (r[j][0] + r[j][1]) + (r[j][2] + r[j][3]);
  }
  const float mean = wave_sum(s) / (float)C;
  float q = 0.f;
#pragma unroll
  for (int j = 0; j < NV; ++j) {
    const int v = lane + 64 * j;
    if (v < nv) {
      const f32x4 d = r[j] - mean;
      q += (d[0] * d[0] + d[1] * d[1]) + (d[2] * d[2] + d[3] * d[3]);
    }
  }
  const float rstd = 1.0f / sqrtf(wave_sum(q) / (float)C + eps);
#pragma unroll
  for (int j = 0; j < NV; ++j) {
    const int v = lane + 64 * j;
    if (v < nv) {
      f32x4 y = (r[j] - mean) * rstd;
      if (gamma) y *= *(const f32x4*)(gamma + v * 4);
      if (beta) y += *(const f32x4*)(beta + v * 4);
      if (act == INK_ACT_GELU) {
#pragma unroll
        for (int e = 0; e < 4; ++e) y[e] = gelu_erf(y[e]);
      }
      if (out_h && split) split_store(out_h + row * ldo + v * 4, C, y);
      else if (out_h) *(f16x4*)(out_h + row * ldo + v * 4) = (f16x4){(f16)y[0], (f16)y[1], (f16)y[2], (f16)y[3]};
      if (out_f) *(f32x4*)(out_f + row * ldf + v * 4) = y;
    }
  }
}

__global__ __launch_bounds__(256) void add_split_f16_kernel(const float* __restrict__ a,
                                                            const float* __restrict__ b,
                                                            f16* __restrict__ o, int64_t n4, int64_t nb4,
                                                            int C) {
  const int c4n = C >> 2;
  for (int64_t i = blockIdx.x * 256 + threadIdx.x; i < n4; i += (int64_t)gridDim.x * 256) {
    f32x4 v = *(const f32x4*)(a + i * 4);
    if (b) v += *(const f32x4*)(b + (i % nb4) * 4);
    const int64_t row = i / c4n;
    const int c = (int)(i - row * c4n) * 4;
    split_store(o + row * 3 * C + c, C, v);
  }
}

__global__ __launch_bounds__(256) void add_cvt_f16_kernel(const float* __restrict__ a,
                                                          const float* __restrict__ b,
                                                          f16* __restrict__ o,
                                                          float* __restrict__ of, int64_t n4,
                                                          int64_t nb4) {
  for (int64_t i = blockIdx.x * 256 + threadIdx.x; i < n4; i += (int64_t)gridDim.x * 256) {
    f32x4 v = *(const f32x4*)(a + i * 4);
    if (b) v += *(const f32x4*)(b + (i % nb4) * 4);
    if (o) *(f16x4*)(o + i * 4) = (f16x4){(f16)v[0], (f16)v[1], (f16)v[2], (f16)v[3]};
    if (of) *(f32x4*)(of + i * 4) = v;
  }
}

}

extern "C" int ink_layernorm_rows(const float* x, int64_t ldx, const float* gamma,
                                  const float* beta, float eps, const int32_t* gather,
                                  int32_t rows_out, int32_t C, void* out_f16, float* out_f32,
                                  int64_t ldo, int32_t act, int32_t split, const float* add, int64_t ld_add,
                                  const int32_t* add_batch_rows, int32_t rows_per_batch, void* stream) {
  INK_CHECK_ARG(x && (out_f16 || out_f32));
  INK_CHECK_ARG(!add || (!gather && rows_per_batch > 0 && ld_add >= C && ld_add % 4 == 0));
  INK_CHECK_ARG(split == 0 || (split == 1 && out_f16 && ldo >= 3 * (int64_t)C && (!out_f32 || ldo % 12 == 0)));
  INK_CHECK_ARG(act == INK_ACT_NONE || act == INK_ACT_GELU);
  INK_CHECK_ARG(rows_out > 0 && C > 0 && C % 4 == 0 && C <= 2048);
  INK_CHECK_ARG(ldx % 4 == 0 && ldo % 4 == 0 && ldx >= C && ldo >= C);
  const dim3 grid((rows_out + 3) / 4), block(256);
  hipStream_t s = (hipStream_t)stream;
  const int nv = (C / 4 + 63) / 64;
#define INK_LN(NV)                                                                          \
  hipLaunchKernelGGL(layernorm_rows_kernel<NV>, grid, block, 0, s, x, ldx, gamma, beta, eps, \
                     gather, rows_out, C, (f16*)out_f16, out_f32, ldo, act, split, add, ld_add, add_batch_rows, \
                     rows_per_batch)
  switch (nv) {
    case 1: INK_LN(1); break;
    case 2: INK_LN(2); break;
    case 3: INK_LN(3); break;
    case 4: INK_LN(4); break;
    case 5: INK_LN(5); break;
    default: INK_LN(8); break;
  }
#undef INK_LN
  return ink_launch_status();
}

extern "C" int ink_add_cvt_f16(const float* a, const float* b, int64_t n_b, void* out_f16,
                               int64_t n, void* stream) {
  INK_CHECK_ARG(a && out_f16 && n > 0 && n % 4 == 0);
  INK_CHECK_ARG(!b || (n_b > 0 && n_b % 4 == 0 && n % n_b == 0));
  const int64_t n4 = n / 4;
  const int blocks = (int)((n4 + 255) / 256 < 2048 ? (n4 + 255) / 256 : 2048);
  hipLaunchKernelGGL(add_cvt_f16_kernel, dim3(blocks), dim3(256), 0, (hipStream_t)stream, a, b,
                     (f16*)out_f16, (float*)nullptr, n4, b ? n_b / 4 : 1);
  return ink_launch_status();
}

extern "C" int ink_add_split_f16(const float* a, const float* b, int64_t n_b, void* out_f16, int64_t n,
                                 int32_t C, void* stream) {
  INK_CHECK_ARG(a && out_f16 && n > 0 && C > 0 && C % 4 == 0 && n % C == 0);
  INK_CHECK_ARG(!b || (n_b > 0 && n_b % 4 == 0 && n % n_b == 0));
  const int64_t n4 = n / 4;
  const int blocks = (int)((n4 + 255) / 256 < 4096 ? (n4 + 255) / 256 : 4096);
  hipLaunchKernelGGL(add_split_f16_kernel, dim3(blocks), dim3(256), 0, (hipStream_t)stream, a, b,
                     (f16*)out_f16, n4, b ? n_b / 4 : 1, C);
  return ink_launch_status();
}

extern "C" int ink_add_f32(const float* a, const float* b, int64_t n_b, float* out, int64_t n,
                           void* stream) {
  INK_CHECK_ARG(a && out && n > 0 && n % 4 == 0);
  INK_CHECK_ARG(!b || (n_b > 0 && n_b % 4 == 0 && n % n_b == 0));
  const int64_t n4 = n / 4;
  const int blocks = (int)((n4 + 255) / 256 < 2048 ? (n4 + 255) / 256 : 2048);
  hipLaunchKernelGGL(add_cvt_f16_kernel, dim3(blocks), dim3(256), 0, (hipStream_t)stream, a, b,
// ... 4 lines not shown
```

### inklayer_amd/ops.py

```python
from __future__ import annotations

import ctypes as C
from typing import Optional, Sequence, Tuple

import torch

from . import _lib
from ._lib import InkAttn, InkGemm, check

ACT = {None: 0, "none": 0, "gelu": 1, "relu": 2}
F16, F32 = torch.float16, torch.float32


_GEMM_TRACE = None


def set_gemm_trace(lst) -> None:
    global _GEMM_TRACE
    _GEMM_TRACE = lst


_ATTN_TRACE = None


def set_attn_trace(lst) -> None:
    global _ATTN_TRACE
    _ATTN_TRACE = lst


def tracing_off() -> bool:
    return _GEMM_TRACE is None and _ATTN_TRACE is None


_raw_stream = getattr(torch._C, "_cuda_getCurrentRawStream", None)
_cur_device = getattr(torch._C, "_cuda_getDevice", None)


def _stream() -> int:
    if _raw_stream is not None and _cur_device is not None:
        return _raw_stream(_cur_device())
    return torch.cuda.current_stream().cuda_stream


def own_f32(t: torch.Tensor, dev) -> torch.Tensor:
    t = t.detach().to(dev, F32).contiguous()
    if t.untyped_storage().nbytes() > t.numel() * t.element_size():
        t = t.clone()
    return t


def _p(t: Optional[torch.Tensor]) -> Optional[int]:
    if t is None:
        return None
    assert t.is_cuda, "InkLayer HIP ops need GPU tensors (no CPU fallback)"
    return t.data_ptr()


def gemm(a: torch.Tensor, w: torch.Tensor, bias: Optional[torch.Tensor] = None, *,
         act: Optional[str] = None, residual: Optional[torch.Tensor] = None,
         col_scale: Optional[torch.Tensor] = None, row_map: Optional[torch.Tensor] = None,
         out: Optional[torch.Tensor] = None, out_dtype: torch.dtype = F32,
         out_rows: Optional[int] = None) -> torch.Tensor:
    assert a.dtype == F16 and w.dtype == F16
    assert a.dim() == 2 and w.dim() == 2 and a.stride(1) == 1 and w.stride(1) == 1
    M, K = a.shape
    N = w.shape[0]
    assert w.shape[1] == K
    p = InkGemm()
    if out is None:
        rows = out_rows if out_rows is not None else M
        out = torch.empty((rows, N), device=a.device, dtype=out_dtype)
    assert out.dim() == 2 and out.stride(1) == 1 and out.shape[1] == N
    p.A, p.W, p.C = a.data_ptr(), w.data_ptr(), out.data_ptr()
    p.bias, p.col_scale = _p(bias), _p(col_scale)
    p.residual, p.row_map = _p(residual), _p(row_map)
    if bias is not None:
        assert bias.dtype == F32 and bias.numel() == N
    if col_scale is not None:
        assert col_scale.dtype == F32 and col_scale.numel() == N
    if residual is not None:
        assert residual.dtype == F32 and residual.stride(1) == 1 and residual.shape[1] == N
        p.ldr = residual.stride(0)
    if row_map is not None:
        assert row_map.dtype == torch.int32 and row_map.numel() == M
    p.M, p.N, p.K = M, N, K
    p.lda, p.ldw, p.ldc = a.stride(0), w.stride(0), out.stride(0)
    p.act = ACT[act]
    p.c_f16 = 1 if out.dtype == F16 else 0
    assert out.dtype in (F16, F32)
    if _GEMM_TRACE is None:
        check(_lib.lib().ink_gemm_f16(C.byref(p), _stream()), "ink_gemm_f16")
    else:
        e0, e1 = torch.cuda.Event(enable_timing=True), torch.cuda.Event(enable_timing=True)
        e0.record()
        check(_lib.lib().ink_gemm_f16(C.byref(p), _stream()), "ink_gemm_f16")
        e1.record()
        _GEMM_TRACE.append((2.0 * M * N * K, e0, e1, (M, N, K, act or '-', 'res' if residual is not None else '-',
                                                      'map' if row_map is not None else '-', 'f16' if p.c_f16 else 'f32')))
    return out


def layernorm_rows(x: torch.Tensor, gamma: Optional[torch.Tensor], beta: Optional[torch.Tensor],
                   eps: float, *, gather: Optional[torch.Tensor] = None,
                   out_dtype: torch.dtype = F16, out: Optional[torch.Tensor] = None,
                   out2: Optional[torch.Tensor] = None, act: Optional[str] = None,
                   split: bool = False, add: Optional[torch.Tensor] = None,
                   add_batch_rows: Optional[torch.Tensor] = None, rows_per_batch: int = 0,
                   split_f32: Optional[torch.Tensor] = None) -> torch.Tensor:
    assert x.dtype == F32 and x.dim() == 2 and x.stride(1) == 1
    Cdim = x.shape[1]
    rows = gather.numel() if gather is not None else x.shape[0]
    wcols = 3 * Cdim if split else Cdim
    if split:
        assert out_dtype == F16 and out2 is None
    if out is None:
        out = torch.empty((rows, wcols), device=x.device, dtype=out_dtype)
    assert out.shape == (rows, wcols) and out.stride(1) == 1
    oh = out.data_ptr() if out.dtype == F16 else None
    of = out.data_ptr() if out.dtype == F32 else None
    if out2 is not None:
        assert out2.shape == out.shape and out2.stride(0) == out.stride(0) and out2.dtype != out.dtype
        if out2.dtype == F16:
            oh = out2.data_ptr()
        else:
            of = out2.data_ptr()
    if split_f32 is not None:
        assert split and out.stride(0) == 3 * Cdim and split_f32.dtype == F32 and split_f32.is_contiguous()
        assert tuple(split_f32.shape) == (rows, Cdim)
        of = split_f32.data_ptr()
    if gather is not None:
        assert gather.dtype == torch.int32
    if add is not None:
        assert gather is None and add.dtype == F32 and add.dim() == 2 and add.stride(1) == 1 and add.shape[1] == Cdim
        if add_batch_rows is not None:
            assert add_batch_rows.dtype == torch.int32 and add_batch_rows.is_cuda and rows_per_batch > 0
            assert add_batch_rows.numel() * rows_per_batch == rows
        else:
            rows_per_batch = rows
    check(_lib.lib().ink_layernorm_rows(x.data_ptr(), x.stride(0), _p(gamma), _p(beta), eps,
                                        _p(gather), rows, Cdim, oh, of, out.stride(0), ACT[act], int(split),
                                        _p(add), add.stride(0) if add is not None else 0, _p(add_batch_rows),
                                        rows_per_batch, _stream()), "ink_layernorm_rows")
    return out


def add_cvt_f16(a: torch.Tensor, b: Optional[torch.Tensor] = None,
                out: Optional[torch.Tensor] = None) -> torch.Tensor:
    assert a.dtype == F32 and a.is_contiguous()
    nb = 0
    if b is not None:
        assert b.dtype == F32 and b.is_contiguous() and a.numel() % b.numel() == 0
        nb = b.numel()
    if out is None:
        out = torch.empty(a.shape, device=a.device, dtype=F16)
    assert out.dtype == F16 and out.is_contiguous() and out.numel() == a.numel()
    check(_lib.lib().ink_add_cvt_f16(a.data_ptr(), _p(b), nb, out.data_ptr(), a.numel(), _stream()),
          "ink_add_cvt_f16")
    return out


def add_split_f16(a: torch.Tensor, b: Optional[torch.Tensor] = None) -> torch.Tensor:
    assert a.dtype == F32 and a.is_contiguous() and a.dim() == 2
    nb = 0
    if b is not None:
        assert b.dtype == F32 and b.is_contiguous() and a.numel() % b.numel() == 0
        nb = b.numel()
    R, Cn = a.shape
    out = torch.empty((R, 3 * Cn), device=a.device, dtype=F16)
    check(_lib.lib().ink_add_split_f16(a.data_ptr(), _p(b), nb, out.data_ptr(), a.numel(), Cn, _stream()),
          "ink_add_split_f16")
    return out


def split_weight(w32: torch.Tensor) -> torch.Tensor:
    w32 = w32.to(torch.float32)
    hi = w32.to(F16)
    lo = ((w32 - hi.to(torch.float32)) * 64.0).to(F16)
    return torch.cat([hi, (hi.to(torch.float32) / 64.0).to(F16), lo], dim=-1).contiguous()


def add_f32(a: torch.Tensor, b: torch.Tensor, out: Optional[torch.Tensor] = None) -> torch.Tensor:
    assert a.dtype == F32 and b.dtype == F32 and a.is_contiguous() and b.is_contiguous()
    assert a.numel() % b.numel() == 0
    if out is None:
        out = torch.empty(a.shape, device=a.device, dtype=F32)
    assert out.is_contiguous() and out.numel() == a.numel()
    check(_lib.lib().ink_add_f32(a.data_ptr(), b.data_ptr(), b.numel(), out.data_ptr(), a.numel(),
                                 _stream()), "ink_add_f32")
    return out


def flash_attn(q: torch.Tensor, k: torch.Tensor, v: torch.Tensor, *, n_batch: int, n_heads: int,
               head_dim: int, scale: float, n_q: Optional[int] = None, n_k: Optional[int] = None,
               rel_h: Optional[torch.Tensor] = None, rel_w: Optional[torch.Tensor] = None,
               rel_aug: Optional[torch.Tensor] = None, grid_w: int = 0,
               dense_bias: Optional[torch.Tensor] = None, dense_mask: Optional[torch.Tensor] = None,
               q_batch_rows: Optional[torch.Tensor] = None,
               kv_batch_rows: Optional[torch.Tensor] = None,
               tok_rows: Optional[torch.Tensor] = None, pad_k: Optional[torch.Tensor] = None,
               pad_v: Optional[torch.Tensor] = None,
               out: Optional[torch.Tensor] = None) -> torch.Tensor:
    for t in (q, k, v):
        assert t.dtype == F16 and t.dim() == 2 and t.stride(1) == 1 and t.is_cuda
    if n_q is None:
        n_q = q.shape[0] // n_batch
    if n_k is None:
        n_k = k.shape[0] // n_batch
    if tok_rows is not None:
        assert rel_aug is not None and out is not None and n_q == n_k
        assert tok_rows.dtype == torch.int32 and tok_rows.is_cuda and tok_rows.numel() == n_batch * n_q
        for t in (pad_k, pad_v):
            assert t is not None and t.dtype == F16 and t.is_contiguous() and t.numel() == n_heads * head_dim
        assert out.dtype == F16 and out.stride(1) == 1
        assert out.shape[0] * out.stride(0) * 2 < 2 ** 31 and q.shape[0] * q.stride(0) * 2 < 2 ** 32
    else:
        if out is None:
            out = torch.empty((n_batch * n_q, n_heads * head_dim), device=q.device, dtype=F16)
        assert out.dtype == F16 and out.shape[0] == n_batch * n_q and out.stride(1) == 1
    p = InkAttn()
    p.Q, p.K, p.V, p.O = q.data_ptr(), k.data_ptr(), v.data_ptr(), out.data_ptr()
    p.ldq, p.ldk, p.ldv, p.ldo = q.stride(0), k.stride(0), v.stride(0), out.stride(0)
    p.n_batch, p.n_heads, p.n_q, p.n_k, p.head_dim = n_batch, n_heads, n_q, n_k, head_dim
    p.scale = scale
    p.grid_w = grid_w
    for name, t in (("q_batch_rows", q_batch_rows), ("kv_batch_rows", kv_batch_rows)):
        if t is not None:
            assert t.dtype == torch.int32 and t.numel() == n_batch and t.is_cuda
            setattr(p, name, t.data_ptr())
    if dense_bias is not None:
        assert dense_bias.dtype == F32 and dense_bias.is_contiguous() and dense_bias.shape == (n_heads, n_q, 64)
        p.bias_mode, p.dense_bias = 3, dense_bias.data_ptr()
        if dense_mask is not None:
            assert dense_mask.dtype == F32 and dense_mask.is_contiguous() and dense_mask.shape[1:] == (n_q, 64)
            p.dense_mask, p.n_mask = dense_mask.data_ptr(), dense_mask.shape[0]
    elif rel_aug is not None:
        assert rel_aug.dtype == F16 and rel_aug.is_contiguous()
        p.bias_mode, p.rel_aug = 2, rel_aug.data_ptr()
        if tok_rows is not None:
            p.tok_rows, p.pad_k, p.pad_v = tok_rows.data_ptr(), pad_k.data_ptr(), pad_v.data_ptr()
    elif rel_h is not None:
        assert rel_h.dtype == rel_w.dtype and rel_h.dtype in (F32, F16)
        assert rel_h.is_contiguous() and rel_w.is_contiguous()
        p.bias_mode, p.rel_h, p.rel_w = 1, rel_h.data_ptr(), rel_w.data_ptr()
        p.rel_f16 = int(rel_h.dtype == F16)
    else:
        p.bias_mode = 0
    if _ATTN_TRACE is None:
        check(_lib.lib().ink_flash_attn(C.byref(p), _stream()), "ink_flash_attn")
    else:
        e0, e1 = torch.cuda.Event(enable_timing=True), torch.cuda.Event(enable_timing=True)
        e0.record()
        check(_lib.lib().ink_flash_attn(C.byref(p), _stream()), "ink_flash_attn")
# ... 424 lines not shown
    assert x.dtype == F32 and x.is_contiguous() and out.dtype == F32
    Cn = x.shape[1]
    ws = torch.empty(B * G * 2, device=x.device, dtype=F32)
    check(_lib.lib().ink_groupnorm_nhwc(x.data_ptr(), B, T, Cn, G, gamma.data_ptr(), beta.data_ptr(), eps,
                                        ws.data_ptr(), out.data_ptr(), out_batch_stride, _stream()),
          "ink_groupnorm_nhwc")


def gather_rows(x: torch.Tensor, idx: torch.Tensor, B: int, rows_per_batch: int, *, x_batch_rows: int,
                idx_batch_stride: int, out_dtype=F16, out: Optional[torch.Tensor] = None) -> torch.Tensor:
    assert x.dtype == F32 and x.stride(1) == 1 and idx.dtype == torch.int32 and idx.is_cuda
    Cn = x.shape[1]
    if out is None:
        out = torch.empty((B * rows_per_batch, Cn), device=x.device, dtype=out_dtype)
    out_dtype = out.dtype
    assert out_dtype in (F16, F32) and out.is_contiguous() and tuple(out.shape) == (B * rows_per_batch, Cn)
    oh = out.data_ptr() if out_dtype == F16 else None
    of = out.data_ptr() if out_dtype == F32 else None
    check(_lib.lib().ink_gather_rows(x.data_ptr(), x.stride(0), x_batch_rows, idx.data_ptr(), idx_batch_stride,
                                     rows_per_batch, B, Cn, oh, of, _stream()), "ink_gather_rows")
    return out


def biattn_fusion(qv16: torch.Tensor, kl16: torch.Tensor, B: int, S: int, T: int, scale: float,
                  chunk: int = 128):
    assert qv16.dtype == F16 and qv16.is_contiguous() and kl16.dtype == F16 and kl16.is_contiguous()
    E = qv16.shape[1] // 2
    dev = qv16.device
    nchunk = -(-S // chunk)
    scores = torch.empty(B * S * 4 * T, device=dev, dtype=F32)
    stats = torch.empty(B * 4 * T * 2, device=dev, dtype=F32)
    partial = torch.empty(B * 4 * nchunk * T * 256, device=dev, dtype=F32)
    out_v = torch.empty((B * S, E), device=dev, dtype=F16)
    out_l = torch.empty((B * T, E), device=dev, dtype=F16)
    check(_lib.lib().ink_biattn_fusion(qv16.data_ptr(), kl16.data_ptr(), B, S, T, E, scale, scores.data_ptr(),
                                       stats.data_ptr(), partial.data_ptr(), chunk, out_v.data_ptr(),
                                       out_l.data_ptr(), _stream()), "ink_biattn_fusion")
    return out_v, out_l


def fusion_fold(v: torch.Tensor, B: int, S: int, lnv_g: torch.Tensor, lnv_b: torch.Tensor, eps: float,
                text_kv: torch.Tensor, T: int, Wqv: torch.Tensor, bqv: torch.Tensor, Wo: torch.Tensor, bo: torch.Tensor,
                gamma_v: torch.Tensor, scale: float, pos: Optional[torch.Tensor] = None,
                out16_pos: Optional[torch.Tensor] = None, out16: Optional[torch.Tensor] = None) -> torch.Tensor:
    for t in (out16, out16_pos):
        assert t is None or (t.dtype == F16 and t.is_contiguous() and tuple(t.shape) == (B * S, 256))
    assert out16_pos is None or (pos is not None and pos.dtype == F32 and pos.is_contiguous() and tuple(pos.shape) == (S, 256))
    assert v.dtype == F32 and v.is_contiguous() and tuple(v.shape) == (B * S, 256)
    assert text_kv.dtype == F32 and text_kv.stride(1) == 1 and tuple(text_kv.shape) == (B * T, 2048)
    assert Wqv.dtype == F16 and Wqv.is_contiguous() and tuple(Wqv.shape) == (2048, 256) and bqv.dtype == F32
    assert Wo.dtype == F16 and Wo.is_contiguous() and tuple(Wo.shape) == (256, 1024)
    need = C.c_int64(0)
    check(_lib.lib().ink_fusion_fold_workspace(B, S, C.byref(need)), "ink_fusion_fold_workspace")
    ws = torch.empty(need.value, device=v.device, dtype=F32)
    out_l = torch.empty((B * T, 1024), device=v.device, dtype=F16)
    check(_lib.lib().ink_fusion_fold(v.data_ptr(), B, S, lnv_g.data_ptr(), lnv_b.data_ptr(), eps, text_kv.data_ptr(),
                                     text_kv[:, 1024:].data_ptr(), text_kv.stride(0), T, Wqv.data_ptr(), bqv.data_ptr(),
                                     Wqv[1024:].data_ptr(), bqv[1024:].data_ptr(), Wo.data_ptr(), bo.data_ptr(),
                                     gamma_v.data_ptr(), scale, ws.data_ptr(), out_l.data_ptr(), _p(pos), _p(out16_pos),
                                     _p(out16), _stream()),
          "ink_fusion_fold")
    return out_l


def proj256_ln_pack(ws: torch.Tensor) -> torch.Tensor:
    assert ws.dtype == F16 and ws.is_contiguous() and tuple(ws.shape) == (256, 384)
    blob = torch.empty(3 * 64 * 64 * 8, device=ws.device, dtype=F16)
    check(_lib.lib().ink_proj256_ln_pack(ws.data_ptr(), blob.data_ptr(), _stream()), "ink_proj256_ln_pack")
    return blob


def proj256_ln(a: torch.Tensor, blob: torch.Tensor, bias: torch.Tensor, res: torch.Tensor, ln_g: torch.Tensor,
               ln_b: torch.Tensor, eps: float, *, res_batch_rows: Optional[torch.Tensor] = None, rows_per_batch: int = 0,
               want_f32: bool = True, want_split: bool = True):
    R = int(a.shape[0])
    assert a.dtype == F32 and a.is_contiguous() and tuple(a.shape) == (R, 128)
    assert blob.dtype == F16 and blob.numel() == 3 * 64 * 64 * 8
    assert res.dtype == F32 and res.is_contiguous() and res.shape[1] == 256
    assert all(t.dtype == F32 and t.is_contiguous() and t.numel() == 256 for t in (bias, ln_g, ln_b))
    if res_batch_rows is not None:
        assert res_batch_rows.dtype == torch.int32 and res_batch_rows.is_cuda and rows_per_batch > 0
        assert res_batch_rows.numel() * rows_per_batch == R
    else:
        assert res.shape[0] == R
    of = torch.empty((R, 256), device=a.device, dtype=F32) if want_f32 else None
    osp = torch.empty((R, 768), device=a.device, dtype=F16) if want_split else None
    check(_lib.lib().ink_proj256_ln(a.data_ptr(), blob.data_ptr(), bias.data_ptr(), res.data_ptr(), _p(res_batch_rows),
                                    rows_per_batch, ln_g.data_ptr(), ln_b.data_ptr(), eps, R, _p(of), _p(osp), _stream()),
          "ink_proj256_ln")
    return of, osp


def sam_upscale_pack(ws: torch.Tensor) -> torch.Tensor:
    assert ws.dtype == F16 and ws.is_contiguous() and tuple(ws.shape) == (128, 192)
    blob = torch.empty(4 * 12 * 64 * 8, device=ws.device, dtype=F16)
    check(_lib.lib().ink_sam_upscale_pack(ws.data_ptr(), blob.data_ptr(), _stream()), "ink_sam_upscale_pack")
    return blob


def sam_upscale_tail(u0: torch.Tensor, n: int, g: int, ln_g: torch.Tensor, ln_b: torch.Tensor, eps: float,
                     blob: torch.Tensor, b3: torch.Tensor, hyper: torch.Tensor) -> torch.Tensor:
    if u0.shape[1] == 64:
        assert u0.is_contiguous() and u0.shape[0] == n * g * g * 4
        u0 = u0.view(n * g * g, 256)
    assert u0.dtype == F32 and u0.stride(1) == 1 and tuple(u0.shape) == (n * g * g, 256) and u0.stride(0) % 4 == 0
    assert blob.dtype == F16 and blob.numel() == 4 * 12 * 64 * 8 and b3.dtype == F32 and b3.numel() == 128
    assert hyper.dtype == F32 and hyper.is_contiguous() and hyper.dim() == 3 and hyper.shape[0] == n and hyper.shape[2] == 32
    assert ln_g.dtype == F32 and ln_b.dtype == F32 and ln_g.numel() == 64 and ln_b.numel() == 64
    M = hyper.shape[1]
    low = torch.empty((n, M, 4 * g, 4 * g), device=u0.device, dtype=F32)
    check(_lib.lib().ink_sam_upscale_tail(_p(u0), u0.stride(0), n, g, _p(ln_g), _p(ln_b), eps, _p(blob), _p(b3), _p(hyper), M,
                                          _p(low), _stream()), "ink_sam_upscale_tail")
    return low


def ffn256_pack(w1: torch.Tensor, b1: torch.Tensor, w2: torch.Tensor, w_pre: Optional[torch.Tensor] = None) -> torch.Tensor:
    hid = int(w1.shape[0])
    assert w1.dtype == F16 and w2.dtype == F16 and w1.is_contiguous() and w2.is_contiguous()
    assert tuple(w1.shape) == (hid, 256) and tuple(w2.shape) == (256, hid)
    assert b1.dtype == F32 and b1.is_contiguous() and b1.numel() == hid
    assert w_pre is None or (w_pre.dtype == F16 and w_pre.is_contiguous() and tuple(w_pre.shape) == (256, 256))
    need = C.c_int64(0)
    check(_lib.lib().ink_ffn256_pack_bytes(hid, int(w_pre is not None), C.byref(need)), "ink_ffn256_pack_bytes")
    blob = torch.empty(need.value // 2, device=w1.device, dtype=F16)
    check(_lib.lib().ink_ffn256_pack(w1.data_ptr(), b1.data_ptr(), w2.data_ptr(), hid, _p(w_pre), blob.data_ptr(), _stream()),
          "ink_ffn256_pack")
    return blob


def ffn256_fused(x16: torch.Tensor, res: torch.Tensor, blob: torch.Tensor, hid: int, b2: torch.Tensor,
                 ln_g: torch.Tensor, ln_b: torch.Tensor, eps: float, out: Optional[torch.Tensor] = None,
                 pre: Optional[Tuple[torch.Tensor, torch.Tensor, torch.Tensor]] = None) -> torch.Tensor:
    M = int(x16.shape[0])
    assert x16.dtype == F16 and x16.stride(1) == 1 and x16.shape[1] == 256
    assert res.dtype == F32 and res.is_contiguous() and tuple(res.shape) == (M, 256)
    need = C.c_int64(0)
    check(_lib.lib().ink_ffn256_pack_bytes(hid, int(pre is not None), C.byref(need)), "ink_ffn256_pack_bytes")
    assert blob.dtype == F16 and blob.numel() * 2 == need.value and b2.dtype == F32
    assert b2.numel() == 256 and ln_g.numel() == 256 and ln_b.numel() == 256 and ln_g.dtype == F32 and ln_b.dtype == F32
    if pre is not None:
        assert all(t.dtype == F32 and t.is_contiguous() and t.numel() == 256 for t in pre)
    if out is None:
        out = torch.empty_like(res)
    assert out.dtype == F32 and out.is_contiguous() and tuple(out.shape) == (M, 256)
    pb, pg, pe = pre if pre is not None else (None, None, None)
    check(_lib.lib().ink_ffn256_fused(x16.data_ptr(), x16.stride(0), res.data_ptr(), blob.data_ptr(), b2.data_ptr(),
                                      ln_g.data_ptr(), ln_b.data_ptr(), eps, M, hid, _p(pb), _p(pg), _p(pe), out.data_ptr(),
                                      _stream()), "ink_ffn256_fused")
    return out


def attn_fewkeys(q: torch.Tensor, k: torch.Tensor, v: torch.Tensor, *, B: int, n_heads: int, head_dim: int,
                 scale: float, blocked: Optional[torch.Tensor] = None, n_q: Optional[int] = None,
                 q_batch_rows: Optional[torch.Tensor] = None, q_add: Optional[torch.Tensor] = None) -> torch.Tensor:
    io = q.dtype
    for t in (q, k, v):
        assert t.dtype == io and io in (F16, F32) and t.dim() == 2 and t.stride(1) == 1
        assert t.data_ptr() % 16 == 0
    if n_q is None:
        n_q = q.shape[0] // B
    n_k = k.shape[0] // B
    out = torch.empty((B * n_q, n_heads * head_dim), device=q.device, dtype=io)
    if blocked is not None:
        assert blocked.dtype == torch.uint8 and blocked.is_contiguous() and blocked.shape == (n_q, n_k)
    if q_batch_rows is not None:
        assert q_batch_rows.dtype == torch.int32 and q_batch_rows.numel() == B and q_batch_rows.is_cuda
    if q_add is not None:
        assert q_add.dtype == F32 and q_add.is_contiguous() and tuple(q_add.shape) == (n_q, n_heads * head_dim)
    check(_lib.lib().ink_attn_fewkeys(q.data_ptr(), q.stride(0), k.data_ptr(), k.stride(0), v.data_ptr(),
                                      v.stride(0), B, n_q, n_k, n_heads, head_dim, scale, _p(blocked),
                                      _p(q_batch_rows), _p(q_add), int(io == F32), out.data_ptr(), out.stride(0), _stream()),
          "ink_attn_fewkeys")
    return out


def attn_fewq(q: torch.Tensor, k: torch.Tensor, v: torch.Tensor, *, n_batch: int, n_heads: int, head_dim: int,
              scale: float, n_q: int, n_k: int, q_batch_rows: Optional[torch.Tensor] = None,
              kv_batch_rows: Optional[torch.Tensor] = None, k_add: Optional[torch.Tensor] = None) -> torch.Tensor:
    for t in (q, k, v):
        assert t.dtype == F32 and t.dim() == 2 and t.stride(1) == 1
        assert t.data_ptr() % 16 == 0
    for rows in (q_batch_rows, kv_batch_rows):
        assert rows is None or (rows.dtype == torch.int32 and rows.numel() == n_batch and rows.is_cuda)
    out = torch.empty((n_batch * n_q, n_heads * head_dim), device=q.device, dtype=F32)
    if k_add is not None:
        assert k_add.dtype == F32 and k_add.is_contiguous() and tuple(k_add.shape) == (n_k, n_heads * head_dim)
    check(_lib.lib().ink_attn_fewq(q.data_ptr(), q.stride(0), k.data_ptr(), k.stride(0), v.data_ptr(), v.stride(0),
                                   n_batch, n_q, n_k, n_heads, head_dim, scale, _p(q_batch_rows),
                                   _p(kv_batch_rows), _p(k_add), out.data_ptr(), out.stride(0), _stream()),
          "ink_attn_fewq")
    return out


def topk_rowmax(logits: torch.Tensor, K: int, want_values: bool = False):
    assert logits.dtype == F32 and logits.is_contiguous() and logits.dim() == 3
    B, S, T = logits.shape
    idx = torch.empty((B, K), device=logits.device, dtype=torch.int32)
    val = torch.empty((B, K), device=logits.device, dtype=F32) if want_values else None
    nchunk = -(-S // 16384)
    ws = torch.empty((B * nchunk * K,), device=logits.device, dtype=torch.int64) if nchunk > 1 else None
    check(_lib.lib().ink_topk_rowmax(logits.data_ptr(), B, S, T, K, idx.data_ptr(), _p(val), _p(ws), _stream()),
          "ink_topk_rowmax")
    return (idx, val) if want_values else idx


def sine_embed4(ref: torch.Tensor, dim_t: torch.Tensor, out: Optional[torch.Tensor] = None) -> torch.Tensor:
    assert ref.dtype == F32 and ref.is_contiguous() and ref.shape[-1] == 4 and dim_t.numel() == 128
    N = ref.numel() // 4
    if out is None:
        out = torch.empty((N, 512), device=ref.device, dtype=F16)
    assert out.dtype == F16 and out.is_contiguous() and tuple(out.shape) == (N, 512)
    check(_lib.lib().ink_sine_embed4(ref.data_ptr(), dim_t.data_ptr(), N, out.data_ptr(), _stream()),
          "ink_sine_embed4")
    return out


def box_refine(delta: torch.Tensor, ref: torch.Tensor, ref_is_logit: bool = False,
               out: Optional[torch.Tensor] = None) -> torch.Tensor:
    assert delta.dtype == F32 and delta.stride(1) == 1 and ref.dtype == F32 and ref.is_contiguous()
    N = ref.numel() // 4
    if out is None:
        out = torch.empty_like(ref)
    assert out.dtype == F32 and out.is_contiguous() and out.shape == ref.shape
    check(_lib.lib().ink_box_refine(delta.data_ptr(), delta.stride(0), ref.data_ptr(), N, int(ref_is_logit),
                                    out.data_ptr(), _stream()), "ink_box_refine")
    return out


def mask_cleanup(masks_u8: torch.Tensor, k: int, area_threshold: int = 500, aspect_threshold: float = 1.1,
                 out: Optional[torch.Tensor] = None) -> torch.Tensor:
    assert masks_u8.dtype == torch.uint8 and masks_u8.is_cuda and masks_u8.is_contiguous() and masks_u8.dim() == 3
    n, H, W = masks_u8.shape
    if out is None:
        out = torch.empty_like(masks_u8)
    if n == 0:
        return out
    assert out.dtype == torch.uint8 and out.is_contiguous() and out.shape == masks_u8.shape
    need = C.c_int64(0)
    check(_lib.lib().ink_mask_cleanup_workspace_ints(n, H, W, k, C.byref(need)), "ink_mask_cleanup_workspace_ints")
    ws = torch.empty(need.value, device=masks_u8.device, dtype=torch.int32)
    ta, tb = torch.empty_like(masks_u8), torch.empty_like(masks_u8)
    check(_lib.lib().ink_mask_cleanup(masks_u8.data_ptr(), n, H, W, k, area_threshold, float(aspect_threshold),
                                      ta.data_ptr(), tb.data_ptr(), ws.data_ptr(), out.data_ptr(), _stream()),
          "ink_mask_cleanup")
    out._ink_overflow_flag = ws[:1]
    return out


def mask_sketch_iou_counts(masks_u8: torch.Tensor, sketch_rgb_u8: torch.Tensor) -> torch.Tensor:
    assert masks_u8.dtype == torch.uint8 and masks_u8.is_cuda and masks_u8.is_contiguous() and masks_u8.dim() == 3
    n, H, W = masks_u8.shape
    assert sketch_rgb_u8.dtype == torch.uint8 and sketch_rgb_u8.is_cuda and sketch_rgb_u8.is_contiguous()
    assert tuple(sketch_rgb_u8.shape) == (H, W, 3), "masks and sketch have the same size on this path"
    counts = torch.empty((n, n, 2), device=masks_u8.device, dtype=torch.int32)
    if n == 0:
        return counts
    bits = torch.empty((n, (H * W + 63) // 64), device=masks_u8.device, dtype=torch.int64)
    check(_lib.lib().ink_mask_sketch_iou_counts(masks_u8.data_ptr(), sketch_rgb_u8.data_ptr(), n, H, W,
                                                bits.data_ptr(), counts.data_ptr(), _stream()),
          "ink_mask_sketch_iou_counts")
    return counts


def depth_patchify(image_u8: torch.Tensor, nh: int, nw: int, P: int, KP: int, mean: Sequence[float],
                   std: Sequence[float], chan_reverse: bool) -> torch.Tensor:
    assert image_u8.dtype == torch.uint8 and image_u8.is_cuda and image_u8.is_contiguous() and image_u8.shape[2] == 3
    H, W = int(image_u8.shape[0]), int(image_u8.shape[1])
    out = torch.empty(((nh // P) * (nw // P), 3 * KP), device=image_u8.device, dtype=F16)
    check(_lib.lib().ink_depth_patchify(image_u8.data_ptr(), H, W, nh, nw, P, KP, (C.c_double * 3)(*mean),
                                        (C.c_double * 3)(*std), int(chan_reverse), out.data_ptr(), _stream()),
          "ink_depth_patchify")
    return out


def resize_bilinear_ac(x: torch.Tensor, B: int, h: int, w: int, H: int, W: int, out_dtype=F32) -> torch.Tensor:
    assert x.dtype == F32 and x.is_contiguous() and x.shape[0] == B * h * w
    Cn = x.shape[1]
    out = torch.empty((B * H * W, Cn), device=x.device, dtype=out_dtype)
    check(_lib.lib().ink_resize_bilinear_ac_nhwc(x.data_ptr(), B, h, w, Cn, H, W,
                                                 out.data_ptr() if out_dtype == F32 else None,
                                                 out.data_ptr() if out_dtype == F16 else None, _stream()),
          "ink_resize_bilinear_ac_nhwc")
    return out


def im2col3x3_ex(x: torch.Tensor, B: int, H: int, W: int, stride: int = 1, relu: bool = False) -> torch.Tensor:
    assert x.dtype == F16 and x.is_contiguous() and x.shape[0] == B * H * W
    Cn = x.shape[1]
    OH, OW = (H - 1) // stride + 1, (W - 1) // stride + 1
    out = torch.empty((B * OH * OW, 9 * Cn), device=x.device, dtype=F16)
    check(_lib.lib().ink_im2col3x3_ex_f16(x.data_ptr(), B, H, W, Cn, stride, int(relu), out.data_ptr(), _stream()),
          "ink_im2col3x3_ex_f16")
    return out


def _planes_like(n: int, H: int, W: int, dev) -> torch.Tensor:
    return torch.empty((n, H, (W + 63) // 64), device=dev, dtype=torch.int64)


def _check_planes(p: torch.Tensor, W: int):
    assert p.dtype == torch.int64 and p.is_cuda and p.is_contiguous() and p.dim() == 3 and p.shape[2] == (W + 63) // 64
    return int(p.shape[0]), int(p.shape[1])


def layers_otsu_planes(gray_u8: torch.Tensor, invert: bool = True) -> Tuple[torch.Tensor, torch.Tensor, torch.Tensor]:
    assert gray_u8.dtype == torch.uint8 and gray_u8.is_cuda and gray_u8.is_contiguous() and gray_u8.dim() == 3
    n, H, W = (int(v) for v in gray_u8.shape)
    dev = gray_u8.device
    hist = torch.empty((n, 256), device=dev, dtype=torch.int32)
    thresh = torch.empty(n, device=dev, dtype=torch.int32)
    planes = _planes_like(n, H, W, dev)
    check(_lib.lib().ink_layers_otsu_planes(gray_u8.data_ptr(), n, H, W, int(invert), hist.data_ptr(), thresh.data_ptr(),
                                            planes.data_ptr(), _stream()), "ink_layers_otsu_planes")
    return planes, hist, thresh


def layers_dilate(planes: torch.Tensor, W: int, kernel_size: int, iterations: int) -> torch.Tensor:
    n, H = _check_planes(planes, W)
    if iterations <= 0:
        return planes.clone()
    tmp, out = torch.empty_like(planes), torch.empty_like(planes)
    check(_lib.lib().ink_layers_dilate(planes.data_ptr(), n, H, W, kernel_size, iterations, tmp.data_ptr(), out.data_ptr(),
                                       _stream()), "ink_layers_dilate")
    return out


# ... 219 lines not shown
```

### inklayer_amd/sam.py

```python
from __future__ import annotations

import math
from dataclasses import dataclass
from typing import Dict, List, Optional, Sequence, Tuple

import numpy as np
import torch

from . import ops
from ._lru import LRU

F16, F32 = torch.float16, torch.float32


@dataclass
class SamConfig:
    embed_dim: int = 1280
    depth: int = 32
    num_heads: int = 16
    global_attn_indexes: Tuple[int, ...] = (7, 15, 23, 31)
    window_size: int = 14
    img_size: int = 1024
    patch_size: int = 16
    mlp_ratio: float = 4.0
# ... 139 lines not shown
        self.T = g * g
        assert E == 256 and (self.T * 4) % 32 == 0, \
            "the fused decoder kernels (csrc/proj_ln.hip, csrc/upscale_tail.hip) are built for SAM's widths"
        self.scale = 80 ** -0.5
        sd = state_dict
        dev = self.dev

        def h(name):
            return sd[name].detach().to(torch.float32).to(dev, F16).contiguous()

        def f(name):
            return ops.own_f32(sd[name], dev)

        def ws(name, shape=None):
            t = sd[name].detach().to(dev, torch.float32)
            return ops.split_weight(t if shape is None else shape(t))

        self.w: Dict[str, torch.Tensor] = {}
        w = self.w
        P = cfg.patch_size
        w["pe.ws"] = ws("image_encoder.patch_embed.proj.weight", lambda t: t.reshape(D, 3 * P * P))
        w["pe.b"] = f("image_encoder.patch_embed.proj.bias")
        w["pos"] = f("image_encoder.pos_embed").reshape(self.T, D).contiguous()
        for i in range(cfg.depth):
            p = f"image_encoder.blocks.{i}."
            for n in ("norm1.weight", "norm1.bias", "norm2.weight", "norm2.bias", "attn.qkv.bias",
                      "attn.proj.bias", "mlp.lin1.bias", "mlp.lin2.bias", "attn.rel_pos_h",
                      "attn.rel_pos_w"):
                w[f"b{i}.{n}"] = f(p + n)
            for n in ("attn.qkv.weight", "attn.proj.weight", "mlp.lin1.weight", "mlp.lin2.weight"):
                w[f"b{i}.{n}"] = h(p + n)
            if i not in cfg.global_attn_indexes:
                qb = w[f"b{i}.attn.qkv.bias"]
                w[f"b{i}.pad_k"] = qb[D:2 * D].to(F16).contiguous()
                w[f"b{i}.pad_v"] = qb[2 * D:].to(F16).contiguous()
        w["neck0.ws"] = ws("image_encoder.neck.0.weight", lambda t: t.reshape(E, D))
        w["neck1.w"], w["neck1.b"] = f("image_encoder.neck.1.weight"), f("image_encoder.neck.1.bias")
        w["neck2.ws"] = ws("image_encoder.neck.2.weight", lambda t: t.permute(0, 2, 3, 1).reshape(E, 9, E)) \
            .reshape(E, 27 * E).contiguous()
        w["neck3.w"], w["neck3.b"] = f("image_encoder.neck.3.weight"), f("image_encoder.neck.3.bias")

        w["gauss"] = f("prompt_encoder.pe_layer.positional_encoding_gaussian_matrix")
        w["no_mask"] = f("prompt_encoder.no_mask_embed.weight").reshape(-1).contiguous()
        w["pt_emb"] = torch.cat([f(f"prompt_encoder.point_embeddings.{i}.weight") for i in range(4)], 0).contiguous()
        if "prompt_encoder.not_a_point_embed.weight" in sd:
            w["not_a_point"] = f("prompt_encoder.not_a_point_embed.weight").reshape(-1).contiguous()
        md = "prompt_encoder.mask_downscaling."
        md_names = ("0.weight", "0.bias", "1.weight", "1.bias", "3.weight", "3.bias", "4.weight", "4.bias", "6.weight",
                    "6.bias")
        if all(md + n in sd for n in md_names):
            w["mask_ds"] = torch.cat([sd[md + n].detach().to(torch.float32).reshape(-1) for n in md_names]) \
                .to(dev).contiguous()
        ar = (torch.arange(g, dtype=torch.float32) + 0.5) / g
        grid_xy = torch.stack([ar[None, :].expand(g, g), ar[:, None].expand(g, g)], -1).reshape(-1, 2)
        self.dense_pe = ops.sam_pe_encode(grid_xy.contiguous().to(dev), w["gauss"])

        t = "mask_decoder.transformer."
        def attn(dst, src):
            for n in ("q_proj", "k_proj", "v_proj", "out_proj"):
                w[f"{dst}.{n}.ws"] = ws(f"{src}.{n}.weight")
                w[f"{dst}.{n}.b"] = f(f"{src}.{n}.bias")

        def cat(dst, names):
            for sfx in (".ws", ".b"):
                w[dst + sfx] = torch.cat([w[n + sfx] for n in names]).contiguous()

        pe_split = ops.add_split_f16(self.dense_pe)
        for i in range(cfg.dec_depth):
            p, d = f"{t}layers.{i}.", f"d{i}"
            attn(d + ".self", p + "self_attn")
            attn(d + ".t2i", p + "cross_attn_token_to_image")
            attn(d + ".i2t", p + "cross_attn_image_to_token")
            if i == 0:
                cat(d + ".self.qkv", [f"{d}.self.{n}" for n in ("q_proj", "k_proj", "v_proj")])
            else:
                cat(d + ".self.qk", [f"{d}.self.{n}" for n in ("q_proj", "k_proj")])
            for n in ("norm1", "norm2", "norm3", "norm4"):
                w[f"{d}.{n}.w"], w[f"{d}.{n}.b"] = f(p + n + ".weight"), f(p + n + ".bias")
            w[d + ".lin1.ws"], w[d + ".lin1.b"] = ws(p + "mlp.lin1.weight"), f(p + "mlp.lin1.bias")
            w[d + ".lin2.ws"], w[d + ".lin2.b"] = ws(p + "mlp.lin2.weight"), f(p + "mlp.lin2.bias")
            cat(d + ".kvq", [d + ".t2i.k_proj", d + ".t2i.v_proj", d + ".i2t.q_proj"])
            w[d + ".t2i.k_pe"] = ops.gemm(pe_split, w[d + ".t2i.k_proj.ws"]).contiguous()
            w[d + ".i2t.q_pe"] = ops.gemm(pe_split, w[d + ".i2t.q_proj.ws"]).contiguous()
            w[d + ".i2t.out_proj.blob"] = ops.proj256_ln_pack(w[d + ".i2t.out_proj.ws"].contiguous())
        attn("dfin", t + "final_attn_token_to_image")
        w["dfin.norm.w"], w["dfin.norm.b"] = f(t + "norm_final_attn.weight"), f(t + "norm_final_attn.bias")
        w["dfin.k_pe"] = ops.gemm(pe_split, w["dfin.k_proj.ws"]).contiguous()
        w["out_tok"] = torch.cat([f("mask_decoder.iou_token.weight"),
                                  f("mask_decoder.mask_tokens.weight")], 0).contiguous()
        u = "mask_decoder.output_upscaling."
        w["up0.ws"] = ws(u + "0.weight", lambda t: t.permute(2, 3, 1, 0).reshape(4 * (E // 4), E))
        w["up0.b"] = f(u + "0.bias").repeat(4).contiguous()
        w["up1.w"], w["up1.b"] = f(u + "1.weight"), f(u + "1.bias")
        up3 = ws(u + "3.weight", lambda t: t.permute(2, 3, 1, 0).reshape(4 * (E // 8), E // 4))
        assert tuple(up3.shape) == (128, 192)
        w["up3.blob"] = ops.sam_upscale_pack(up3.contiguous())
        w["up3.b"] = f(u + "3.bias").repeat(4).contiguous()
        cat("dfin.kvu", ["dfin.k_proj", "dfin.v_proj", "up0"])
        for j in range(3):
            w[f"iou{j}.ws"] = ws(f"mask_decoder.iou_prediction_head.layers.{j}.weight")
            w[f"iou{j}.b"] = f(f"mask_decoder.iou_prediction_head.layers.{j}.bias")
            for m in range(cfg.num_mask_tokens):
                hk = f"mask_decoder.output_hypernetworks_mlps.{m}.layers.{j}."
                if m == 0 or hk + "bias" in sd:
                    w[f"{_hyp(m)}{j}.b"] = f(hk + "bias")
                if m == 0 or hk + "weight" in sd:
                    w[f"{_hyp(m)}{j}.ws"] = ws(hk + "weight")

        self._alloc(max_batch)
        if bias_correction:
            self._calibrate_bias_correction(sd)

    @torch.no_grad()
    def _calibrate_bias_correction(self, sd) -> None:
        cfg, w, D = self.cfg, self.w, self.cfg.embed_dim
        page = torch.full((cfg.img_size, cfg.img_size, 3), 255, dtype=torch.uint8, device=self.dev)
        means: Dict[str, torch.Tensor] = {}
        self._calib = means
        try:
            self.encode([page])
        finally:
            self._calib = None
        for i in range(cfg.depth):
            p = f"image_encoder.blocks.{i}."
            for lin in ("attn.qkv", "mlp.lin1", "attn.proj", "mlp.lin2"):
                W32 = sd[p + lin + ".weight"].detach().to(self.dev, torch.float32)
                w16, bkey = w[f"b{i}.{lin}.weight"], f"b{i}.{lin}.bias"
                w[bkey] = (w[bkey].double() + (W32 - w16.float()).double() @ means[f"b{i}.{lin}"].double()).float().contiguous()

    def _alloc(self, B: int) -> None:
        cfg, dev, T, D = self.cfg, self.dev, self.T, self.cfg.embed_dim
        g, ws = cfg.grid, cfg.window_size
        self.max_batch = B
        nwin = -(-g // ws)
        self.nwin = nwin
        Mw = nwin * nwin * ws * ws
        self.Mw = Mw
        self._enc_graphs = LRU(self.graph_cache_size)
        self._enc_seen: Dict[int, int] = {}
        self.win_map = window_rows(B, g, ws).to(dev)
        P = cfg.patch_size
        e = lambda *s, dt=F16: torch.empty(s, device=dev, dtype=dt)
        self.buf_patches = e(B * T, 3 * P * P * 3)
        self.x = e(B * T, D, dt=F32)
        self.pos_rep = self.w["pos"].repeat(B, 1).contiguous()
        self.y = e(B * T, D)
        self.qkv = e(B * T, 3 * D)
        self.att = e(B * T, D)
        self.hid = e(B * T, int(D * cfg.mlp_ratio))
        H = cfg.num_heads
        self.rel_aug = e(B * nwin * nwin * H * ws * ws, 32)
        self.rel_h = e(B * H * T, 64)
        self.rel_w = e(B * H * T, 64)

    def encode(self, images_u8: Sequence[torch.Tensor], chan_reverse: bool = False,
               upto: Optional[int] = None) -> torch.Tensor:
        cfg, w, T, D = self.cfg, self.w, self.T, self.cfg.embed_dim
        B = len(images_u8)
        assert 1 <= B <= self.max_batch
        H, Mw = cfg.num_heads, self.Mw
        x = self.x[:B * T]
        for b, img in enumerate(images_u8):
            ops.sam_patchify(img, cfg.img_size, cfg.patch_size, cfg.pixel_mean, cfg.pixel_std,
                             chan_reverse, self.buf_patches[b * T:(b + 1) * T], split=True)
        ops.gemm(self.buf_patches[:B * T], w["pe.ws"], w["pe.b"], residual=self.pos_rep[:B * T], out=x)
        if upto is None and self.graph_blocks and ops.tracing_off():
            return self._blocks_graphed(B)
        return self._blocks(B, upto)

    graph_blocks = False
    graph_cache_size = 2

    def _blocks_graphed(self, B: int) -> torch.Tensor:
        g = self._enc_graphs.get(B)
        if g is None:
            self._enc_seen[B] = self._enc_seen.get(B, 0) + 1
            if self._enc_seen[B] < 2:
                return self._blocks(B, None)
            x0 = self.x[:B * self.T].clone()
            cur = torch.cuda.current_stream(self.dev)
            side = torch.cuda.Stream(device=self.dev)
            side.wait_stream(cur)
            with torch.cuda.stream(side):
                self._blocks(B, None)
                self.x[:B * self.T].copy_(x0)
            cur.wait_stream(side)
            graph = torch.cuda.CUDAGraph()
            with torch.cuda.graph(graph):
                out = self._blocks(B, None)
            self.x[:B * self.T].copy_(x0)
            g = (graph, out)
            self._enc_graphs.put(B, g)
        g[0].replay()
        return g[1].clone()

    def _blocks(self, B: int, upto: Optional[int]) -> torch.Tensor:
        cfg, w, T, D = self.cfg, self.w, self.T, self.cfg.embed_dim
        H, Mw = cfg.num_heads, self.Mw
        x = self.x[:B * T]
        nblk = cfg.depth if upto is None else upto
        calib = getattr(self, "_calib", None)
        for i in range(nblk):
            k = f"b{i}."
            y = ops.layernorm_rows(x, w[k + "norm1.weight"], w[k + "norm1.bias"], 1e-6, out=self.y[:B * T])
            if calib is not None:
                calib[k + "attn.qkv"] = y.float().mean(0)
            qkv = ops.gemm(y, w[k + "attn.qkv.weight"], w[k + "attn.qkv.bias"], out=self.qkv[:B * T])
            q, kk, v = qkv[:, :D], qkv[:, D:2 * D], qkv[:, 2 * D:]
            if i in cfg.global_attn_indexes:
                rh, rw = ops.relpos_bias(q, w[k + "attn.rel_pos_h"], w[k + "attn.rel_pos_w"], S=cfg.grid,
                                         n_batch=B, n_heads=H, head_dim=80, scale=self.scale,
                                         out=(self.rel_h, self.rel_w), f16_tables=True)
                o = ops.flash_attn(q, kk, v, n_batch=B, n_heads=H, head_dim=80, scale=self.scale,
                                   rel_h=rh, rel_w=rw, grid_w=cfg.grid, out=self.att[:B * T])
            else:
                wm = self.win_map[:B * Mw]
                nb = B * self.nwin * self.nwin
                aug = ops.relpos_bias(q, w[k + "attn.rel_pos_h"], w[k + "attn.rel_pos_w"],
                                      S=cfg.window_size, n_batch=nb, n_heads=H, head_dim=80,
                                      scale=self.scale, out=self.rel_aug, tok_rows=wm)
                o = ops.flash_attn(q, kk, v, n_batch=nb, n_heads=H, head_dim=80, scale=self.scale,
                                   n_q=cfg.window_size ** 2, n_k=cfg.window_size ** 2,
                                   rel_aug=aug, grid_w=cfg.window_size, tok_rows=wm,
                                   pad_k=w[k + "pad_k"], pad_v=w[k + "pad_v"], out=self.att[:B * T])
            if calib is not None:
                calib[k + "attn.proj"] = o.float().mean(0)
            ops.gemm(o, w[k + "attn.proj.weight"], w[k + "attn.proj.bias"], residual=x, out=x)
            y = ops.layernorm_rows(x, w[k + "norm2.weight"], w[k + "norm2.bias"], 1e-6, out=self.y[:B * T])
            hd = ops.gemm(y, w[k + "mlp.lin1.weight"], w[k + "mlp.lin1.bias"], act="gelu", out=self.hid[:B * T])
            if calib is not None:
                calib[k + "mlp.lin1"], calib[k + "mlp.lin2"] = y.float().mean(0), hd.float().mean(0)
            ops.gemm(hd, w[k + "mlp.lin2.weight"], w[k + "mlp.lin2.bias"], residual=x, out=x)
        if upto is not None:
            return x.view(B, T, D)
        n0 = ops.gemm(ops.add_split_f16(x), w["neck0.ws"])
        n1 = ops.layernorm_rows(n0, w["neck1.w"], w["neck1.b"], 1e-6, split=True)
        n2 = ops.gemm(ops.im2col3x3(n1, B, cfg.grid, cfg.grid), w["neck2.ws"])
        emb = ops.layernorm_rows(n2, w["neck3.w"], w["neck3.b"], 1e-6, out_dtype=F32)
        return emb.view(B, T, cfg.prompt_embed_dim)

    def decode(self, emb: torch.Tensor, boxes_input_frame: np.ndarray | torch.Tensor,
               input_hw: Tuple[int, int], orig_hw: Tuple[int, int], want_logits: bool = False):
        boxes = torch.as_tensor(np.asarray(boxes_input_frame), dtype=torch.float32).reshape(-1, 4)
        low, iou = self.decode_low_res(emb.reshape(1, self.T, -1), boxes, [0] * boxes.shape[0])
        res = ops.sam_postprocess(low, self.cfg.img_size, input_hw, orig_hw, self.cfg.mask_threshold, want_logits)
        if want_logits:
            return res[0], low, iou, res[1]
        return res

    def decode_low_res(self, emb: torch.Tensor, boxes: torch.Tensor, img_of_box: Sequence[int]):
        low, iou = self.decode_prompts(emb, img_of_box, boxes=boxes)
        return low.view(low.shape[0], *low.shape[-2:]), iou

    def decode_prompts(self, emb: torch.Tensor, img_of_prompt: Sequence[int], points: Optional[torch.Tensor] = None,
                       labels: Optional[torch.Tensor] = None, boxes: Optional[torch.Tensor] = None,
                       mask_input: Optional[torch.Tensor] = None, multimask_output: bool = False,
                       masks: Optional[Tuple[int, int]] = None):
        cfg, w, dev, L = self.cfg, self.w, self.dev, self.cfg.img_size
        P, _ = check_prompts(points, labels, boxes, mask_input, mask_side=4 * cfg.grid)
        if len(img_of_prompt) != P or not all(0 <= int(i) < emb.shape[0] for i in img_of_prompt):
            raise ValueError(f"img_of_prompt must name an image of emb for each of the {P} prompts")
        lo, M = masks if masks is not None else ((1, 3) if multimask_output else (0, 1))
        if M not in (1, 3, 4) or not 0 <= lo <= cfg.num_mask_tokens - M:
            raise ValueError(f"masks=(first, count) must select 1, 3 or 4 of the {cfg.num_mask_tokens} mask tokens")
        need = [("not_a_point", points is not None, "prompt_encoder.not_a_point_embed"),
                ("mask_ds", mask_input is not None, "prompt_encoder.mask_downscaling")]
        need += [(f"{_hyp(m)}0.ws", m > 0, f"mask_decoder.output_hypernetworks_mlps.{m}") for m in range(lo, lo + M)]
        missing = [name for key, used, name in need if used and key not in w]
        if missing:
            raise ValueError(f"these prompts need weights the engine's state dict did not have: {missing}")

        def dev32(t, dt=F32):
            t = torch.as_tensor(t)
            return t.to(dev, dt).contiguous() if t.is_cuda else _to_dev_async(t.to(dt), dev)

        pts = lab = bx = None
        if points is not None:
            pts, lab = dev32(points), dev32(labels, torch.int32)
        if boxes is not None:
            bx = dev32(torch.as_tensor(boxes).reshape(-1, 4))
        tokens = ops.sam_prompt_tokens(w["gauss"], w["pt_emb"], w.get("not_a_point", w["no_mask"]), w["out_tok"],
                                       float(L), P, points=pts, labels=lab, boxes=bx,
                                       pad=points is not None and boxes is None)
        mi = dev32(mask_input) if mask_input is not None else None
        return self._decode_tokens_split(emb, tokens, img_of_prompt, mask_input=mi, mask_lo=lo, n_masks=M)

    def _decode_tokens_split(self, emb: torch.Tensor, tokens: torch.Tensor, img_of_box: Sequence[int],
                             mask_input: Optional[torch.Tensor] = None, mask_lo: int = 0, n_masks: int = 1):
        cfg, w, T, dev = self.cfg, self.w, self.T, self.dev
        E, g = cfg.prompt_embed_dim, cfg.grid
        B = emb.shape[0]
        n, NT = tokens.shape[0], tokens.shape[1]
        assert n > 0 and len(img_of_box) == n and NT <= MAX_TOKENS
        Hh = cfg.dec_heads
        SP = ops.add_split_f16

        def lin(x_split, name, bias=True, **kw):
            return ops.gemm(x_split, w[name + ".ws"], w[name + ".b"] if bias else None, **kw)

        qpe = tokens.view(n * NT, E)
        iob = torch.as_tensor(list(img_of_box), dtype=torch.int64)
        img_rows = _to_dev_async((iob * T).to(torch.int32), dev)
        if mask_input is None:
            keys = ops.add_f32(emb.reshape(B * T, E).contiguous(), w["no_mask"])
            shared = True
            ks = None
        else:
            keys, ks = ops.sam_mask_embed(mask_input, emb.reshape(B * T, E).contiguous(), img_rows, w["mask_ds"], 1e-6,
                                          split=True)
            shared = False
        queries = qpe
        sc32, sc16 = 1.0 / math.sqrt(32), 1.0 / math.sqrt(16)

        Eh = E // 2

        def t2i_attend(name, queries, k, v, k_pe, residual):
            q = lin(SP(queries, qpe), name + ".q_proj")
            a = ops.attn_fewq(q, k, v, n_batch=n, n_heads=Hh, head_dim=16, scale=sc16, n_q=NT, n_k=T,
                              kv_batch_rows=img_rows if shared else None, k_add=k_pe)
            return lin(SP(a), name + ".out_proj", residual=residual)

        for i in range(cfg.dec_depth):
            d = f"d{i}"
            if i == 0:
                qkv = ops.gemm(SP(queries), w[d + ".self.qkv.ws"], w[d + ".self.qkv.b"])
                a = ops.attn_fewkeys(qkv[:, :E], qkv[:, E:2 * E], qkv[:, 2 * E:], B=n, n_heads=Hh, head_dim=32,
                                     scale=sc32)
                queries = lin(SP(a), d + ".self.out_proj")
            else:
                qk = ops.gemm(SP(queries, qpe), w[d + ".self.qk.ws"], w[d + ".self.qk.b"])
                v = lin(SP(queries), d + ".self.v_proj")
                a = ops.attn_fewkeys(qk[:, :E], qk[:, E:], v, B=n, n_heads=Hh, head_dim=32, scale=sc32)
                queries = lin(SP(a), d + ".self.out_proj", residual=queries)
            queries = ops.layernorm_rows(queries, w[d + ".norm1.w"], w[d + ".norm1.b"], 1e-5, out_dtype=F32)
            kvq = ops.gemm(SP(keys) if ks is None else ks, w[d + ".kvq.ws"], w[d + ".kvq.b"])
            queries = ops.layernorm_rows(t2i_attend(d + ".t2i", queries, kvq[:, :Eh], kvq[:, Eh:2 * Eh],
                                                    w[d + ".t2i.k_pe"], queries),
                                         w[d + ".norm2.w"], w[d + ".norm2.b"], 1e-5, out_dtype=F32)
            hmid = lin(SP(queries), d + ".lin1", act="relu")
            queries = ops.layernorm_rows(lin(SP(hmid), d + ".lin2", residual=queries),
                                         w[d + ".norm3.w"], w[d + ".norm3.b"], 1e-5, out_dtype=F32)
            ik = lin(SP(queries, qpe), d + ".i2t.k_proj")
            iv = lin(SP(queries), d + ".i2t.v_proj")
            a = ops.attn_fewkeys(kvq[:, 2 * Eh:], ik, iv, B=n, n_heads=Hh, head_dim=16, scale=sc16, n_q=T,
                                 q_batch_rows=img_rows if shared else None, q_add=w[d + ".i2t.q_pe"])
            last = i + 1 == cfg.dec_depth
            keys, ks = ops.proj256_ln(a, w[d + ".i2t.out_proj.blob"], w[d + ".i2t.out_proj.b"], keys, w[d + ".norm4.w"],
                                      w[d + ".norm4.b"], 1e-5, res_batch_rows=img_rows if shared else None,
                                      rows_per_batch=T if shared else 0, want_f32=not last, want_split=True)
            shared = False
        kvu = ops.gemm(ks, w["dfin.kvu.ws"], w["dfin.kvu.b"])
        kv = kvu[:, :2 * Eh]
        queries = ops.layernorm_rows(t2i_attend("dfin", queries, kv[:, :Eh], kv[:, Eh:], w["dfin.k_pe"], queries),
                                     w["dfin.norm.w"], w["dfin.norm.b"], 1e-5, out_dtype=F32)
        hs = queries.view(n, NT, E)

        def mlp3(prefix: str, x: torch.Tensor) -> torch.Tensor:
            a = lin(SP(x), prefix + "0", act="relu")
            a = lin(SP(a), prefix + "1", act="relu")
            return lin(SP(a), prefix + "2")

        M = n_masks
        if M == 1:
            hyper = mlp3(_hyp(mask_lo), hs[:, 1 + mask_lo].contiguous()).view(n, 1, 32)
        else:
            hyper = torch.stack([mlp3(_hyp(m), hs[:, 1 + m].contiguous()) for m in range(mask_lo, mask_lo + M)], 1)
        iou = mlp3("iou", hs[:, 0].contiguous())[:, mask_lo:mask_lo + M]
        u0 = kvu[:, 2 * Eh:]
        low = ops.sam_upscale_tail(u0, n, g, w["up1.w"], w["up1.b"], 1e-6, w["up3.blob"], w["up3.b"], hyper)
        return low, iou


class SamPredictor:

    def __init__(self, engine: SamEngine):
        self.engine = engine
        self.cfg = engine.cfg
        self.transform = ResizeLongestSide(engine.cfg.img_size)
        self.reset_image()

    def reset_image(self) -> None:
        self.is_image_set = False
        self.features = None
        self.original_size = None
        self.input_size = None

    def set_image(self, image: np.ndarray, image_format: str = "RGB") -> None:
        assert image_format in ("RGB", "BGR")
        if image_format != "RGB":
            image = image[..., ::-1]
        raw = torch.from_numpy(np.ascontiguousarray(image)).to(self.engine.dev)
        nh, nw = preprocess_shape(image.shape[0], image.shape[1], self.cfg.img_size)
        dev_img = ops.resize_bilinear_u8(raw, nh, nw)
        self.original_size = tuple(image.shape[:2])
        self.input_size = (nh, nw)
        self.features = self.engine.encode([dev_img])[0]
        self.is_image_set = True

    def apply_boxes(self, boxes: torch.Tensor) -> torch.Tensor:
        return self.transform.apply_boxes_torch(boxes.detach().cpu(), self.original_size)

    def apply_coords(self, coords: np.ndarray, original_size: Optional[Tuple[int, int]] = None) -> np.ndarray:
        return self.transform.apply_coords(coords, original_size or self.original_size)

    def apply_coords_torch(self, coords: torch.Tensor, original_size: Optional[Tuple[int, int]] = None) -> torch.Tensor:
        return self.transform.apply_coords_torch(coords, original_size or self.original_size)

    def predict(self, point_coords: Optional[np.ndarray] = None, point_labels: Optional[np.ndarray] = None,
                box: Optional[np.ndarray] = None, mask_input: Optional[np.ndarray] = None,
                multimask_output: bool = True, return_logits: bool = False):
        if not self.is_image_set:
            raise RuntimeError("An image must be set with .set_image(...) before mask prediction.")
        if point_coords is not None and point_labels is None:
            raise ValueError("point_labels must be supplied if point_coords is supplied.")
        coords = labels = boxes = mask = None
        if point_coords is not None:
            coords = torch.as_tensor(self.apply_coords(point_coords), dtype=torch.float)[None]
            labels = torch.as_tensor(np.asarray(point_labels), dtype=torch.int)[None]
        if box is not None:
            boxes = torch.as_tensor(self.transform.apply_boxes(box, self.original_size), dtype=torch.float)[:1]
        if mask_input is not None:
            mask = torch.as_tensor(mask_input, dtype=torch.float)[None]
        masks, iou, low = self.predict_torch(coords, labels, boxes, mask, multimask_output, return_logits=return_logits)
        return masks[0].cpu().numpy(), iou[0].cpu().numpy(), low[0].cpu().numpy()

    def predict_torch(self, point_coords=None, point_labels=None, boxes: torch.Tensor = None,
                      mask_input=None, multimask_output: bool = False, return_logits: bool = False):
        if not self.is_image_set:
            raise RuntimeError("An image must be set with .set_image(...) before mask prediction.")
        eng = self.engine
        P, _ = check_prompts(point_coords, point_labels, boxes, mask_input, mask_side=4 * self.cfg.grid)
        low, iou = eng.decode_prompts(self.features.reshape(1, eng.T, -1), [0] * P, point_coords, point_labels, boxes,
                                      mask_input, multimask_output)
        C, S = low.shape[1], low.shape[-1]
        res = ops.sam_postprocess(low.view(P * C, S, S), self.cfg.img_size, self.input_size, self.original_size,
                                  self.cfg.mask_threshold, return_logits)
        out = res[1] if return_logits else res.bool()
        return out.view(P, C, *self.original_size), iou, low


_ENGINES: Dict[str, SamEngine] = {}


def build_sam(checkpoint: Optional[str] = None, state_dict=None, device="cuda",
              max_batch: int = 1) -> SamEngine:
    if state_dict is None:
        if checkpoint in _ENGINES:
            return _ENGINES[checkpoint]
        state_dict = torch.load(checkpoint, map_location="cpu", weights_only=True)
    eng = SamEngine(state_dict, SamConfig(), device, max_batch)
    if checkpoint is not None:
        _ENGINES[checkpoint] = eng
    return eng


def run_SAM(image_pil, boxes_filt: torch.Tensor, sam_checkpoint: Optional[str] = None,
            engine: Optional[SamEngine] = None) -> List[np.ndarray]:
    if len(boxes_filt) == 0:
        return []
    eng = engine if engine is not None else build_sam(sam_checkpoint)
    pred = SamPredictor(eng)
    image = np.array(image_pil)[..., ::-1]
    pred.set_image(np.ascontiguousarray(image))
    tb = pred.apply_boxes(boxes_filt)
    masks, _, _ = pred.predict_torch(None, None, boxes=tb, multimask_output=False)
    m = masks[:, 0].cpu().numpy()
    return [m[i] for i in range(m.shape[0])]


def __getattr__(name):
    if name == "SamAutomaticMaskGenerator":
        from .amg import SamAutomaticMaskGenerator
        return SamAutomaticMaskGenerator
    raise AttributeError(f"module {__name__!r} has no attribute {name!r}")
```

Baseline: 117.8.

## Fuse split-f16 conversion into GEMM/attention epilogues and implicit-im2col neck conv

Adds a split-f16 output (hi, lo, scaled-hi) written directly from the GEMM epilogue, the few-keys attention kernels and layernorm. The SAM mask decoder no longer runs separate SP() split-conversion passes between linears. Adds a tap-row (implicit im2col) mode to the GEMM so the neck 3x3 conv reads layernorm output through a row-index table, with a zero row for padding, instead of materializing an im2col buffer. This removes many small kernel launches and intermediate tensors, at the cost of extra gather indexing in the GEMM A-load path and more epilogue stores.

```diff
diff --git a/include/inklayer_hip.h b/include/inklayer_hip.h
--- a/include/inklayer_hip.h
+++ b/include/inklayer_hip.h
@@ -27,6 +27,14 @@
 #define INK_ACT_GELU 1
 #define INK_ACT_RELU 2
 int ink_gemm_f16(const InkGemm* p, void* stream);
+typedef struct InkGemmEx {
+  const int32_t* a_tap_rows;
+  int32_t a_tap_k;
+  int32_t a_zero_row;
+  void* C_split;
+  int32_t ldcs;
+} InkGemmEx;
+int ink_gemm_f16_ex(const InkGemm* p, const InkGemmEx* ex, void* stream);
 int ink_gemm_set_variant(int32_t v);
 int ink_gemm_query_variant(int32_t M, int32_t N, int32_t K);
 
@@ -143,6 +151,10 @@
                      int32_t B, int32_t n_q, int32_t n_k, int32_t n_heads, int32_t head_dim, float scale,
                      const uint8_t* blocked, const int32_t* q_batch_rows, const float* q_add, int32_t io_f32, void* O,
                      int64_t ldo, void* stream);
+int ink_attn_fewkeys_split(const void* Q, int64_t ldq, const void* K, int64_t ldk, const void* V, int64_t ldv,
+                           int32_t B, int32_t n_q, int32_t n_k, int32_t n_heads, int32_t head_dim, float scale,
+                           const uint8_t* blocked, const int32_t* q_batch_rows, const float* q_add, int32_t io_f32,
+                           void* O, int64_t ldo, void* O_split, int64_t ldos, void* stream);
 
 int ink_attn_fewq(const void* Q, int64_t ldq, const void* K, int64_t ldk, const void* V, int64_t ldv,
                   int32_t n_batch, int32_t n_q, int32_t n_k, int32_t n_heads, int32_t head_dim, float scale,
diff --git a/inklayer_amd/_lib.py b/inklayer_amd/_lib.py
--- a/inklayer_amd/_lib.py
+++ b/inklayer_amd/_lib.py
@@ -17,6 +17,13 @@
         ("M", c_int), ("N", c_int), ("K", c_int),
         ("lda", c_int), ("ldw", c_int), ("ldr", c_int), ("ldc", c_int),
         ("act", c_int), ("c_f16", c_int),
+    ]
+
+
+class InkGemmEx(C.Structure):
+    _fields_ = [
+        ("a_tap_rows", c_void_p), ("a_tap_k", c_int), ("a_zero_row", c_int),
+        ("C_split", c_void_p), ("ldcs", c_int),
     ]
 
 
@@ -36,6 +43,7 @@
 SIGNATURES = {
     "ink_abi_version": [],
     "ink_gemm_f16": [C.POINTER(InkGemm), c_void_p],
+    "ink_gemm_f16_ex": [C.POINTER(InkGemm), C.POINTER(InkGemmEx), c_void_p],
     "ink_gemm_set_variant": [c_int],
     "ink_gemm_query_variant": [c_int, c_int, c_int],
     "ink_layernorm_rows": [c_void_p, c_i64, c_void_p, c_void_p, c_float, c_void_p, c_int, c_int,
@@ -101,6 +109,8 @@
                         c_void_p, c_void_p, c_void_p],
     "ink_attn_fewkeys": [c_void_p, c_i64, c_void_p, c_i64, c_void_p, c_i64, c_int, c_int, c_int, c_int, c_int,
                          c_float, c_void_p, c_void_p, c_void_p, c_int, c_void_p, c_i64, c_void_p],
+    "ink_attn_fewkeys_split": [c_void_p, c_i64, c_void_p, c_i64, c_void_p, c_i64, c_int, c_int, c_int, c_int, c_int,
+                               c_float, c_void_p, c_void_p, c_void_p, c_int, c_void_p, c_i64, c_void_p, c_i64, c_void_p],
     "ink_attn_fewq": [c_void_p, c_i64, c_void_p, c_i64, c_void_p, c_i64, c_int, c_int, c_int, c_int, c_int,
                       c_float, c_void_p, c_void_p, c_void_p, c_void_p, c_i64, c_void_p],
     "ink_topk_rowmax": [c_void_p, c_int, c_int, c_int, c_int, c_void_p, c_void_p, c_void_p, c_void_p],
diff --git a/inklayer_amd/csrc/attn_few.hip b/inklayer_amd/csrc/attn_few.hip
--- a/inklayer_amd/csrc/attn_few.hip
+++ b/inklayer_amd/csrc/attn_few.hip
@@ -32,7 +32,8 @@
                                                            const uint8_t* __restrict__ blocked,
                                                            const int32_t* __restrict__ q_rows,
                                                            const float* __restrict__ q_add,
-                                                           T* __restrict__ O, int64_t ldo) {
+                                                           T* __restrict__ O, int64_t ldo, f16* __restrict__ Os,
+                                                           int64_t ldos) {
   const int64_t gid = (int64_t)blockIdx.x * 256 + threadIdx.x;
   if (gid >= (int64_t)B * n_q * n_heads) return;
   const int h = (int)(gid % n_heads);
@@ -81,9 +82,17 @@
       for (int j = 0; j < 8; ++j) acc[8 * i + j] = fmaf(pw, vv[j], acc[8 * i + j]);
     }
   }
-  T* op = O + bq * ldo + h * HD;
-#pragma unroll
-  for (int i = 0; i < HD / 8; ++i) store8(op + 8 * i, acc + 8 * i);
+  if (O) {
+    T* op = O + bq * ldo + h * HD;
+#pragma unroll
+    for (int i = 0; i < HD / 8; ++i) store8(op + 8 * i, acc + 8 * i);
+  }
+  if (Os) {
+#pragma unroll
+    for (int i = 0; i < HD / 4; ++i)
+      split_store(Os + bq * ldos + h * HD + 4 * i, n_heads * HD,
+                  (f32x4){acc[4 * i], acc[4 * i + 1], acc[4 * i + 2], acc[4 * i + 3]});
+  }
 }
 
 
@@ -94,7 +103,8 @@
                                                                  int n_q, int n_heads, float scale,
                                                                  const int32_t* __restrict__ q_rows,
                                                                  const float* __restrict__ q_add,
-                                                                 float* __restrict__ O, int64_t ldo) {
+                                                                 float* __restrict__ O, int64_t ldo,
+                                                                 f16* __restrict__ Os, int64_t ldos) {
   const int64_t gid = (int64_t)blockIdx.x * 256 + threadIdx.x;
   if (gid >= (int64_t)B * n_q * n_heads * 4) return;
   const int part = (int)(gid & 3);
@@ -130,7 +140,8 @@
   f32x4 acc = {0.f, 0.f, 0.f, 0.f};
 #pragma unroll
   for (int t = 0; t < NK; ++t) acc += (sc[t] * inv) * vv[t];
-  *(f32x4*)(O + bq * ldo + col) = acc;
+  if (O) *(f32x4*)(O + bq * ldo + col) = acc;
+  if (Os) split_store(Os + bq * ldos + col, n_heads * 16, acc);
 }
 
 template <int QW>
@@ -321,22 +332,26 @@
 
 }
 
-extern "C" int ink_attn_fewkeys(const void* Q, int64_t ldq, const void* K, int64_t ldk, const void* V,
-                                int64_t ldv, int32_t B, int32_t n_q, int32_t n_k, int32_t n_heads,
-                                int32_t head_dim, float scale, const uint8_t* blocked,
-                                const int32_t* q_batch_rows, const float* q_add, int32_t io_f32, void* O,
-                                int64_t ldo, void* stream) {
-  INK_CHECK_ARG(Q && K && V && O && B > 0 && n_q > 0 && n_k > 0 && n_k <= 16 && n_heads > 0);
-  INK_CHECK_ARG(ldq % 8 == 0 && ldk % 8 == 0 && ldv % 8 == 0 && ldo % 8 == 0);
+extern "C" int ink_attn_fewkeys_split(const void* Q, int64_t ldq, const void* K, int64_t ldk, const void* V,
+                                      int64_t ldv, int32_t B, int32_t n_q, int32_t n_k, int32_t n_heads,
+                                      int32_t head_dim, float scale, const uint8_t* blocked,
+                                      const int32_t* q_batch_rows, const float* q_add, int32_t io_f32, void* O,
+                                      int64_t ldo, void* O_split, int64_t ldos, void* stream) {
+  INK_CHECK_ARG(Q && K && V && (O || O_split) && B > 0 && n_q > 0 && n_k > 0 && n_k <= 16 && n_heads > 0);
+  INK_CHECK_ARG(ldq % 8 == 0 && ldk % 8 == 0 && ldv % 8 == 0 && (!O || ldo % 8 == 0));
   INK_CHECK_ARG(io_f32 == 0 || io_f32 == 1);
   INK_CHECK_ARG((((uintptr_t)Q | (uintptr_t)K | (uintptr_t)V | (uintptr_t)O) & 15) == 0);
+  INK_CHECK_ARG(!O_split || (io_f32 == 1 && ldos % 8 == 0 && ldos >= 3 * (int64_t)n_heads * head_dim &&
+                             ((uintptr_t)O_split & 15) == 0));
+  f16* Os = (f16*)O_split;
   INK_CHECK_ARG(!q_add || (((uintptr_t)q_add & 15) == 0));
   const int64_t total = (int64_t)B * n_q * n_heads;
   const dim3 grid((unsigned)((total + 255) / 256)), block(256);
   hipStream_t s = (hipStream_t)stream;
 #define INK_FEWKEYS(HD, T)                                                                                     \
   hipLaunchKernelGGL((attn_fewkeys_kernel<HD, T>), grid, block, 0, s, (const T*)Q, ldq, (const T*)K, ldk,      \
-                     (const T*)V, ldv, B, n_q, n_k, n_heads, scale, blocked, q_batch_rows, q_add, (T*)O, ldo)
+                     (const T*)V, ldv, B, n_q, n_k, n_heads, scale, blocked, q_batch_rows, q_add, (T*)O, ldo, Os, \
+                     ldos)
   if (head_dim == 32 && !io_f32) INK_FEWKEYS(32, f16);
   else if (head_dim == 64 && !io_f32) INK_FEWKEYS(64, f16);
   else if (!io_f32) return INK_ERR_ARG;
@@ -346,7 +361,8 @@
 #define INK_FEWKEYS16(NK)                                                                                        \
   case NK:                                                                                                      \
     hipLaunchKernelGGL(attn_fewkeys16_f32_kernel<NK>, g4, block, 0, s, (const float*)Q, ldq, (const float*)K, ldk, \
-                       (const float*)V, ldv, B, n_q, n_heads, scale, q_batch_rows, q_add, (float*)O, ldo);         \
+                       (const float*)V, ldv, B, n_q, n_heads, scale, q_batch_rows, q_add, (float*)O, ldo, Os,     \
+                       ldos);                                                                                    \
     break
     switch (n_k) {
       INK_FEWKEYS16(7); INK_FEWKEYS16(8); INK_FEWKEYS16(9); INK_FEWKEYS16(10); INK_FEWKEYS16(11);
@@ -358,6 +374,16 @@
   else return INK_ERR_ARG;
 #undef INK_FEWKEYS
   return ink_launch_status();
+}
+
+extern "C" int ink_attn_fewkeys(const void* Q, int64_t ldq, const void* K, int64_t ldk, const void* V,
+                                int64_t ldv, int32_t B, int32_t n_q, int32_t n_k, int32_t n_heads,
+                                int32_t head_dim, float scale, const uint8_t* blocked,
+                                const int32_t* q_batch_rows, const float* q_add, int32_t io_f32, void* O,
+                                int64_t ldo, void* stream) {
+  INK_CHECK_ARG(O != nullptr);
+  return ink_attn_fewkeys_split(Q, ldq, K, ldk, V, ldv, B, n_q, n_k, n_heads, head_dim, scale, blocked, q_batch_rows,
+                                q_add, io_f32, O, ldo, nullptr, 0, stream);
 }
 
 extern "C" int ink_attn_fewq(const void* Q, int64_t ldq, const void* K, int64_t ldk, const void* V, int64_t ldv,
diff --git a/inklayer_amd/csrc/common.h b/inklayer_amd/csrc/common.h
--- a/inklayer_amd/csrc/common.h
+++ b/inklayer_amd/csrc/common.h
@@ -47,6 +47,19 @@
   return fmaf(-0.5f * fabsf(x), e, fmaxf(x, 0.0f));
 }
 
+__device__ __forceinline__ void split_store(f16* o, int C, const f32x4& y) {
+  f16x4 hi, lo, hs;
+#pragma unroll
+  for (int e = 0; e < 4; ++e) {
+    hi[e] = (f16)y[e];
+    lo[e] = (f16)((y[e] - (float)hi[e]) * 64.0f);
+    hs[e] = (f16)((float)hi[e] * 0.015625f);
+  }
+  *(f16x4*)o = hi;
+  *(f16x4*)(o + C) = lo;
+  *(f16x4*)(o + 2 * C) = hs;
+}
+
 __device__ __forceinline__ int xcd_remap(int bid, int nwg) {
   const int q = nwg >> 3, r = nwg & 7, x = bid & 7;
   return (x < r ? x * (q + 1) : r * (q + 1) + (x - r) * q) + (bid >> 3);
diff --git a/inklayer_amd/csrc/gemm.hip b/inklayer_amd/csrc/gemm.hip
--- a/inklayer_amd/csrc/gemm.hip
+++ b/inklayer_amd/csrc/gemm.hip
@@ -4,6 +4,13 @@
 #include "../../include/inklayer_hip.h"
 
 namespace {
+
+struct GemmArgs : InkGemm {
+  const int32_t* a_tap_rows;
+  int32_t a_tap_k, a_zero_row;
+  void* C_split;
+  int32_t ldcs;
+};
 
 template <int BK> struct Swz;
 template <> struct Swz<64> {
@@ -16,12 +23,12 @@
 typedef __attribute__((address_space(1))) const void* gptr_t;
 typedef __attribute__((address_space(3))) void* lptr_t;
 
-__device__ __forceinline__ bool residual_preloaded(const InkGemm& p) {
+__device__ __forceinline__ bool residual_preloaded(const GemmArgs& p) {
   return p.residual && p.act == INK_ACT_NONE && !p.col_scale;
 }
 
 template <int TM>
-__device__ __forceinline__ void wave_rows(int (&rows)[TM], const InkGemm& p, int mw, int lane) {
+__device__ __forceinline__ void wave_rows(int (&rows)[TM], const GemmArgs& p, int mw, int lane) {
 #pragma unroll
   for (int ti = 0; ti < TM; ++ti) {
     const int m = mw + ti * 16 + (lane & 15);
@@ -32,7 +39,7 @@
 }
 
 template <int TM, int TN>
-__device__ __forceinline__ void init_wave_tile(f32x4 (&acc)[TM][TN], const InkGemm& p, const int (&rows)[TM], int nw,
+__device__ __forceinline__ void init_wave_tile(f32x4 (&acc)[TM][TN], const GemmArgs& p, const int (&rows)[TM], int nw,
                                                int lane) {
   const int fq = lane >> 4;
   const bool pre = residual_preloaded(p);
@@ -49,7 +56,7 @@
 }
 
 template <int TM, int TN>
-__device__ __forceinline__ void add_bias_wave_tile(f32x4 (&acc)[TM][TN], const InkGemm& p, int nw, int lane) {
+__device__ __forceinline__ void add_bias_wave_tile(f32x4 (&acc)[TM][TN], const GemmArgs& p, int nw, int lane) {
   const int fq = lane >> 4;
 #pragma unroll
   for (int j = 0; j < TN; ++j) {
@@ -62,15 +69,15 @@
 }
 
 template <int TM, int TN, int OUT, int MODE = -1>
-__device__ __forceinline__ void store_wave_tile(f32x4 (&acc)[TM][TN], const InkGemm& p, char* er,
+__device__ __forceinline__ void store_wave_tile(f32x4 (&acc)[TM][TN], const GemmArgs& p, char* er,
                                                 const int (&rows)[TM], int nw, int lane) {
   constexpr bool F16O = OUT == 1;
   constexpr int WNC = TN * 16, EP = WNC * 4 + 16;
-  constexpr int ES = OUT == 0 ? 4 : 8;
+  constexpr int ES = F16O ? 8 : 4;
   constexpr int CPRW = WNC / ES;
   constexpr int NIT = (16 * CPRW + 63) / 64;
   const int fr = lane & 15, fq = lane >> 4;
-  const bool wide16 = OUT != 0 && (p.ldc % 8 == 0);
+  const bool wide16 = F16O && (p.ldc % 8 == 0);
   const bool res_late = MODE < 0 && p.residual && !residual_preloaded(p);
   const int act = MODE < 0 ? p.act : MODE;
   const bool scaled = MODE < 0 && p.col_scale != nullptr;
@@ -131,7 +138,8 @@
         } else {
           f32x4 d = *(const f32x4*)src;
           if (res_late) d += *(const f32x4*)(p.residual + (size_t)r * p.ldr + c_n);
-          *(f32x4*)((float*)p.C + (size_t)r * p.ldc + c_n) = d;
+          if (OUT != 2 || p.C) *(f32x4*)((float*)p.C + (size_t)r * p.ldc + c_n) = d;
+          if (OUT == 2) split_store((f16*)p.C_split + (size_t)r * p.ldcs + c_n, p.N, d);
         }
       }
     }
@@ -152,8 +160,8 @@
 }
 
 constexpr int NS = 2;
-template <int BM, int BN, int BK, int WM, int WN>
-__global__ __launch_bounds__(WM * WN * 64) void gemm_f16_nt(InkGemm p, int group_m) {
+template <int BM, int BN, int BK, int WM, int WN, bool TAPS = false>
+__global__ __launch_bounds__(WM * WN * 64) void gemm_f16_nt(GemmArgs p, int group_m) {
   constexpr int NT = WM * WN * 64;
   constexpr int CPR = BK / 8;
   constexpr int ROWB = BK * 2;
@@ -181,13 +189,27 @@
 
   const f16* srcA[IT_A];
   const f16* srcW[IT_W];
+  const int32_t* tapA[IT_A];
+  int arow[IT_A];
 #pragma unroll
   for (int it = 0; it < IT_A; ++it) {
     const int pch = it * NT + tid;
     const int row = pch / CPR;
     const int lch = (pch % CPR) ^ Swz<BK>::f(row);
-    srcA[it] = A + (size_t)min(m0 + row, p.M - 1) * p.lda + lch * 8;
-  }
+    if (TAPS) {
+      srcA[it] = A + lch * 8;
+      tapA[it] = p.a_tap_rows + min(m0 + row, p.M - 1);
+    } else {
+      srcA[it] = A + (size_t)min(m0 + row, p.M - 1) * p.lda + lch * 8;
+    }
+  }
+  const int ntap = TAPS ? p.K / p.a_tap_k : 1;
+  int tap_nx = 0, kin_nx = 0;
+  auto tap_rows = [&]() {
+    const size_t t = (size_t)min(tap_nx, ntap - 1) * p.M;
+#pragma unroll
+    for (int it = 0; it < IT_A; ++it) arow[it] = tapA[it][t];
+  };
 #pragma unroll
   for (int it = 0; it < IT_W; ++it) {
     const int pch = it * NT + tid;
@@ -199,11 +221,22 @@
   auto stage = [&](int buf, int kt) {
     char* base = smem + buf * STAGE;
 #pragma unroll
-    for (int it = 0; it < IT_A; ++it)
-      __builtin_amdgcn_global_load_lds((gptr_t)(srcA[it] + kt * BK), (lptr_t)(base + (it * NT + wave * 64) * 16), 16, 0, 0);
+    for (int it = 0; it < IT_A; ++it) {
+      const f16* src = srcA[it] + kt * BK;
+      if (TAPS) src = srcA[it] + (size_t)(arow[it] < 0 ? p.a_zero_row : arow[it]) * p.lda + kin_nx;
+      __builtin_amdgcn_global_load_lds((gptr_t)src, (lptr_t)(base + (it * NT + wave * 64) * 16), 16, 0, 0);
+    }
 #pragma unroll
     for (int it = 0; it < IT_W; ++it)
       __builtin_amdgcn_global_load_lds((gptr_t)(srcW[it] + kt * BK), (lptr_t)(base + TILE_A + (it * NT + wave * 64) * 16), 16, 0, 0);
+    if (TAPS) {
+      kin_nx += BK;
+      if (kin_nx == p.a_tap_k) {
+        kin_nx = 0;
+        ++tap_nx;
+      }
+      tap_rows();
+    }
   };
 
   int rows[TM];
@@ -239,6 +272,7 @@
     }
   };
 
+  if (TAPS) tap_rows();
   stage(0, 0);
   init_wave_tile<TM, TN>(acc, p, rows, n0 + wn * (BN / WN), lane);
   for (int kt = 0; kt < nk; ++kt) {
@@ -255,13 +289,15 @@
   char* er = smem + wave * (16 * EP);
   if (p.c_f16 == 1) {
     store_wave_tile<TM, TN, 1>(acc, p, er, rows, n0 + wn * WNC, lane);
+  } else if (p.C_split) {
+    store_wave_tile<TM, TN, 2>(acc, p, er, rows, n0 + wn * WNC, lane);
   } else {
     store_wave_tile<TM, TN, 0>(acc, p, er, rows, n0 + wn * WNC, lane);
   }
 }
 
 constexpr int PP_RING = 4, PP_TN = 5;
-__global__ __launch_bounds__(512) void gemm_f16_nt_pp(InkGemm p, int group_m) {
+__global__ __launch_bounds__(512) void gemm_f16_nt_pp(GemmArgs p, int group_m) {
   constexpr int RING = PP_RING, TN = PP_TN;
   constexpr int BM = 256, BN = 64 * TN, BK = 32, NT = 512;
   constexpr int CPR = BK / 8, ROWB = BK * 2;
@@ -400,7 +436,7 @@
   }
 }
 
-static int launch_gemm_pp(const InkGemm& p, hipStream_t s, int group_m) {
+static int launch_gemm_pp(const GemmArgs& p, hipStream_t s, int group_m) {
   if (p.K / 32 < PP_RING) return INK_ERR_ARG;
   constexpr int BN = 64 * PP_TN;
   constexpr int lds = PP_RING * (256 + BN) * 32 * 2;
@@ -413,15 +449,15 @@
   return ink_launch_status();
 }
 
-template <int BM, int BN, int BK, int WM, int WN>
-static int launch_gemm(const InkGemm& p, hipStream_t s, int group_m = 1) {
+template <int BM, int BN, int BK, int WM, int WN, bool TAPS = false>
+static int launch_gemm(const GemmArgs& p, hipStream_t s, int group_m = 1) {
   constexpr int lds = NS * (BM + BN) * BK * 2;
   static_assert(lds <= 160 * 1024, "LDS budget");
-  static bool attr = ((void)hipFuncSetAttribute((const void*)gemm_f16_nt<BM, BN, BK, WM, WN>,
+  static bool attr = ((void)hipFuncSetAttribute((const void*)gemm_f16_nt<BM, BN, BK, WM, WN, TAPS>,
                                                 hipFuncAttributeMaxDynamicSharedMemorySize, lds), true);
   (void)attr;
   const int ntm = (p.M + BM - 1) / BM, ntn = (p.N + BN - 1) / BN;
-  hipLaunchKernelGGL((gemm_f16_nt<BM, BN, BK, WM, WN>), dim3(ntm * ntn), dim3(WM * WN * 64), lds, s, p, group_m);
+  hipLaunchKernelGGL((gemm_f16_nt<BM, BN, BK, WM, WN, TAPS>), dim3(ntm * ntn), dim3(WM * WN * 64), lds, s, p, group_m);
   return ink_launch_status();
 }
 
@@ -442,26 +478,43 @@
   return INK_OK;
 }
 
-extern "C" int ink_gemm_f16(const InkGemm* pp, void* stream) {
+extern "C" int ink_gemm_f16_ex(const InkGemm* pp, const InkGemmEx* ex, void* stream) {
   INK_CHECK_ARG(pp != nullptr);
-  const InkGemm& p = *pp;
-  INK_CHECK_ARG(p.A && p.W && p.C);
+  GemmArgs p = {};
+  static_cast<InkGemm&>(p) = *pp;
+  if (ex) {
+    p.a_tap_rows = ex->a_tap_rows, p.a_tap_k = ex->a_tap_k, p.a_zero_row = ex->a_zero_row;
+    p.C_split = ex->C_split, p.ldcs = ex->ldcs;
+  }
+  INK_CHECK_ARG(p.A && p.W && (p.C || p.C_split));
   INK_CHECK_ARG(p.M > 0 && p.N > 0 && p.K > 0);
   INK_CHECK_ARG(p.K % 32 == 0 && p.N % 4 == 0);
-  INK_CHECK_ARG(p.lda % 8 == 0 && p.ldw % 8 == 0 && p.lda >= p.K && p.ldw >= p.K);
-  INK_CHECK_ARG(p.ldc % 4 == 0 && p.ldc >= p.N);
+  const bool taps = p.a_tap_rows != nullptr;
+  INK_CHECK_ARG(p.lda % 8 == 0 && p.ldw % 8 == 0 && (taps || p.lda >= p.K) && p.ldw >= p.K);
+  INK_CHECK_ARG(!p.C || (p.ldc % 4 == 0 && p.ldc >= p.N));
+  INK_CHECK_ARG(!p.C_split || (p.c_f16 == 0 && p.ldcs % 4 == 0 && p.ldcs >= 3 * (int64_t)p.N &&
+                               ((uintptr_t)p.C_split & 15) == 0));
   INK_CHECK_ARG(!p.residual || (p.ldr % 4 == 0 && p.ldr >= p.N));
   INK_CHECK_ARG(((uintptr_t)p.A & 15) == 0 && ((uintptr_t)p.W & 15) == 0);
   INK_CHECK_ARG(((uintptr_t)p.C & 15) == 0);
   INK_CHECK_ARG(p.act >= 0 && p.act <= 2);
   INK_CHECK_ARG(p.c_f16 == 0 || p.c_f16 == 1);
+  INK_CHECK_ARG(!taps || (p.a_tap_k > 0 && p.a_tap_k % 64 == 0 && p.K % p.a_tap_k == 0 && p.lda >= p.a_tap_k &&
+                          p.a_zero_row >= 0));
   hipStream_t s = (hipStream_t)stream;
   if (p.K % 64 != 0) return launch_gemm<128, 128, 32, 2, 2>(p, s);
   int v = g_variant;
   if (v < 0) v = ink_gemm_query_variant(p.M, p.N, p.K);
+  if (v == 45 && (taps || p.C_split)) return INK_ERR_ARG;
+  if (taps) {
+    if (v == 10) return launch_gemm<256, 256, 64, 4, 4, true>(p, s, 4);
+    return launch_gemm<128, 128, 64, 2, 2, true>(p, s);
+  }
   switch (v) {
     case 10: return launch_gemm<256, 256, 64, 4, 4>(p, s, 4);
     case 45: return launch_gemm_pp(p, s, 4);
     default: return launch_gemm<128, 128, 64, 2, 2>(p, s);
   }
 }
+
+extern "C" int ink_gemm_f16(const InkGemm* pp, void* stream) { return ink_gemm_f16_ex(pp, nullptr, stream); }
diff --git a/inklayer_amd/csrc/norm.hip b/inklayer_amd/csrc/norm.hip
--- a/inklayer_amd/csrc/norm.hip
+++ b/inklayer_amd/csrc/norm.hip
@@ -2,19 +2,6 @@
 #include "../../include/inklayer_hip.h"
 
 namespace {
-
-__device__ __forceinline__ void split_store(f16* o, int C, const f32x4& y) {
-  f16x4 hi, lo, hs;
-#pragma unroll
-  for (int e = 0; e < 4; ++e) {
-    hi[e] = (f16)y[e];
-    lo[e] = (f16)((y[e] - (float)hi[e]) * 64.0f);
-    hs[e] = (f16)((float)hi[e] * 0.015625f);
-  }
-  *(f16x4*)o = hi;
-  *(f16x4*)(o + C) = lo;
-  *(f16x4*)(o + 2 * C) = hs;
-}
 
 template <int NV>
 __global__ __launch_bounds__(256) void layernorm_rows_kernel(
diff --git a/inklayer_amd/ops.py b/inklayer_amd/ops.py
--- a/inklayer_amd/ops.py
+++ b/inklayer_amd/ops.py
@@ -6,7 +6,7 @@
 import torch
 
 from . import _lib
-from ._lib import InkAttn, InkGemm, check
+from ._lib import InkAttn, InkGemm, InkGemmEx, check
 
 ACT = {None: 0, "none": 0, "gelu": 1, "relu": 2}
 F16, F32 = torch.float16, torch.float32
@@ -60,18 +60,33 @@
          act: Optional[str] = None, residual: Optional[torch.Tensor] = None,
          col_scale: Optional[torch.Tensor] = None, row_map: Optional[torch.Tensor] = None,
          out: Optional[torch.Tensor] = None, out_dtype: torch.dtype = F32,
-         out_rows: Optional[int] = None) -> torch.Tensor:
+         out_rows: Optional[int] = None, taps: Optional[torch.Tensor] = None, split: Optional[str] = None):
     assert a.dtype == F16 and w.dtype == F16
     assert a.dim() == 2 and w.dim() == 2 and a.stride(1) == 1 and w.stride(1) == 1
     M, K = a.shape
     N = w.shape[0]
+    p, ex = InkGemm(), InkGemmEx()
+    if taps is not None:
+        assert taps.dtype == torch.int32 and taps.dim() == 2 and taps.is_contiguous() and taps.device == a.device
+        assert K % 64 == 0, "a tap is whole K-tiles of 64 columns"
+        ex.a_tap_rows, ex.a_tap_k, ex.a_zero_row = taps.data_ptr(), K, M - 1
+        M, K = taps.shape[1], taps.shape[0] * K
     assert w.shape[1] == K
-    p = InkGemm()
-    if out is None:
-        rows = out_rows if out_rows is not None else M
+    assert split in (None, "only", "both")
+    rows = out.shape[0] if out is not None else (out_rows if out_rows is not None else M)
+    osp = None
+    if split:
+        assert out_dtype == F32 and (out is None or split == "both")
+        osp = torch.empty((rows, 3 * N), device=a.device, dtype=F16)
+        ex.C_split, ex.ldcs = osp.data_ptr(), osp.stride(0)
+    if out is None and split != "only":
         out = torch.empty((rows, N), device=a.device, dtype=out_dtype)
-    assert out.dim() == 2 and out.stride(1) == 1 and out.shape[1] == N
-    p.A, p.W, p.C = a.data_ptr(), w.data_ptr(), out.data_ptr()
+    if out is not None:
+        assert out.dim() == 2 and out.stride(1) == 1 and out.shape[1] == N and out.dtype in (F16, F32)
+        assert not (split and out.dtype != F32)
+        p.C, p.ldc = out.data_ptr(), out.stride(0)
+        p.c_f16 = 1 if out.dtype == F16 else 0
+    p.A, p.W = a.data_ptr(), w.data_ptr()
     p.bias, p.col_scale = _p(bias), _p(col_scale)
     p.residual, p.row_map = _p(residual), _p(row_map)
     if bias is not None:
@@ -84,20 +99,31 @@
     if row_map is not None:
         assert row_map.dtype == torch.int32 and row_map.numel() == M
     p.M, p.N, p.K = M, N, K
-    p.lda, p.ldw, p.ldc = a.stride(0), w.stride(0), out.stride(0)
+    p.lda, p.ldw = a.stride(0), w.stride(0)
     p.act = ACT[act]
-    p.c_f16 = 1 if out.dtype == F16 else 0
-    assert out.dtype in (F16, F32)
+    pex = C.byref(ex) if taps is not None or split else None
     if _GEMM_TRACE is None:
-        check(_lib.lib().ink_gemm_f16(C.byref(p), _stream()), "ink_gemm_f16")
+        check(_lib.lib().ink_gemm_f16_ex(C.byref(p), pex, _stream()), "ink_gemm_f16_ex")
     else:
         e0, e1 = torch.cuda.Event(enable_timing=True), torch.cuda.Event(enable_timing=True)
         e0.record()
-        check(_lib.lib().ink_gemm_f16(C.byref(p), _stream()), "ink_gemm_f16")
+        check(_lib.lib().ink_gemm_f16_ex(C.byref(p), pex, _stream()), "ink_gemm_f16_ex")
         e1.record()
         _GEMM_TRACE.append((2.0 * M * N * K, e0, e1, (M, N, K, act or '-', 'res' if residual is not None else '-',
                                                       'map' if row_map is not None else '-', 'f16' if p.c_f16 else 'f32')))
-    return out
+    return {None: out, "only": osp, "both": (out, osp)}[split]
+
+
+def conv3x3_tap_rows(B: int, H: int, W: int) -> torch.Tensor:
+    y = torch.arange(H, dtype=torch.int32).view(1, H, 1)
+    x = torch.arange(W, dtype=torch.int32).view(1, 1, W)
+    b = torch.arange(B, dtype=torch.int32).view(B, 1, 1)
+    t = torch.empty((9, B, H, W), dtype=torch.int32)
+    for k in range(9):
+        yy, xx = y + (k // 3 - 1), x + (k % 3 - 1)
+        inside = (yy >= 0) & (yy < H) & (xx >= 0) & (xx < W)
+        t[k] = torch.where(inside, (b * H + yy) * W + xx, torch.full((), -1, dtype=torch.int32))
+    return t.view(9, B * H * W).contiguous()
 
 
 def layernorm_rows(x: torch.Tensor, gamma: Optional[torch.Tensor], beta: Optional[torch.Tensor],
@@ -828,7 +854,8 @@
 
 def attn_fewkeys(q: torch.Tensor, k: torch.Tensor, v: torch.Tensor, *, B: int, n_heads: int, head_dim: int,
                  scale: float, blocked: Optional[torch.Tensor] = None, n_q: Optional[int] = None,
-                 q_batch_rows: Optional[torch.Tensor] = None, q_add: Optional[torch.Tensor] = None) -> torch.Tensor:
+                 q_batch_rows: Optional[torch.Tensor] = None, q_add: Optional[torch.Tensor] = None,
+                 split: Optional[str] = None):
     io = q.dtype
     for t in (q, k, v):
         assert t.dtype == io and io in (F16, F32) and t.dim() == 2 and t.stride(1) == 1
@@ -836,18 +863,22 @@
     if n_q is None:
         n_q = q.shape[0] // B
     n_k = k.shape[0] // B
-    out = torch.empty((B * n_q, n_heads * head_dim), device=q.device, dtype=io)
+    assert split in (None, "only", "both") and (split is None or io == F32)
+    out = torch.empty((B * n_q, n_heads * head_dim), device=q.device, dtype=io) if split != "only" else None
+    osp = torch.empty((B * n_q, 3 * n_heads * head_dim), device=q.device, dtype=F16) if split else None
     if blocked is not None:
         assert blocked.dtype == torch.uint8 and blocked.is_contiguous() and blocked.shape == (n_q, n_k)
     if q_batch_rows is not None:
         assert q_batch_rows.dtype == torch.int32 and q_batch_rows.numel() == B and q_batch_rows.is_cuda
     if q_add is not None:
         assert q_add.dtype == F32 and q_add.is_contiguous() and tuple(q_add.shape) == (n_q, n_heads * head_dim)
-    check(_lib.lib().ink_attn_fewkeys(q.data_ptr(), q.stride(0), k.data_ptr(), k.stride(0), v.data_ptr(),
-                                      v.stride(0), B, n_q, n_k, n_heads, head_dim, scale, _p(blocked),
-                                      _p(q_batch_rows), _p(q_add), int(io == F32), out.data_ptr(), out.stride(0), _stream()),
-          "ink_attn_fewkeys")
-    return out
+    check(_lib.lib().ink_attn_fewkeys_split(q.data_ptr(), q.stride(0), k.data_ptr(), k.stride(0), v.data_ptr(),
+                                            v.stride(0), B, n_q, n_k, n_heads, head_dim, scale, _p(blocked),
+                                            _p(q_batch_rows), _p(q_add), int(io == F32), _p(out),
+                                            out.stride(0) if out is not None else 0, _p(osp),
+                                            osp.stride(0) if osp is not None else 0, _stream()),
+          "ink_attn_fewkeys_split")
+    return {None: out, "only": osp, "both": (out, osp)}[split]
 
 
 def attn_fewq(q: torch.Tensor, k: torch.Tensor, v: torch.Tensor, *, n_batch: int, n_heads: int, head_dim: int,
diff --git a/inklayer_amd/sam.py b/inklayer_amd/sam.py
--- a/inklayer_amd/sam.py
+++ b/inklayer_amd/sam.py
@@ -315,6 +315,8 @@
         self.rel_aug = e(B * nwin * nwin * H * ws * ws, 32)
         self.rel_h = e(B * H * T, 64)
         self.rel_w = e(B * H * T, 64)
+        self.n1 = torch.zeros((B * T + 1, 3 * cfg.prompt_embed_dim), device=dev, dtype=F16)
+        self._neck_taps: Dict[int, torch.Tensor] = {B: ops.conv3x3_tap_rows(B, g, g).to(dev)}
 
     def encode(self, images_u8: Sequence[torch.Tensor], chan_reverse: bool = False,
                upto: Optional[int] = None) -> torch.Tensor:
@@ -397,8 +399,10 @@
         if upto is not None:
             return x.view(B, T, D)
         n0 = ops.gemm(ops.add_split_f16(x), w["neck0.ws"])
-        n1 = ops.layernorm_rows(n0, w["neck1.w"], w["neck1.b"], 1e-6, split=True)
-        n2 = ops.gemm(ops.im2col3x3(n1, B, cfg.grid, cfg.grid), w["neck2.ws"])
+        ops.layernorm_rows(n0, w["neck1.w"], w["neck1.b"], 1e-6, split=True, out=self.n1[:B * T])
+        if B not in self._neck_taps:
+            self._neck_taps[B] = ops.conv3x3_tap_rows(B, cfg.grid, cfg.grid).to(self.dev)
+        n2 = ops.gemm(self.n1, w["neck2.ws"], taps=self._neck_taps[B])
         emb = ops.layernorm_rows(n2, w["neck3.w"], w["neck3.b"], 1e-6, out_dtype=F32)
         return emb.view(B, T, cfg.prompt_embed_dim)
 
@@ -477,34 +481,38 @@
 
         Eh = E // 2
 
-        def t2i_attend(name, queries, k, v, k_pe, residual):
-            q = lin(SP(queries, qpe), name + ".q_proj")
+        def ln_split(x, name, eps):
+            f = torch.empty_like(x)
+            return f, ops.layernorm_rows(x, w[name + ".w"], w[name + ".b"], eps, split=True, split_f32=f)
+
+        def t2i_attend(name, q_split, k, v, k_pe, residual):
+            q = lin(q_split, name + ".q_proj")
             a = ops.attn_fewq(q, k, v, n_batch=n, n_heads=Hh, head_dim=16, scale=sc16, n_q=NT, n_k=T,
                               kv_batch_rows=img_rows if shared else None, k_add=k_pe)
             return lin(SP(a), name + ".out_proj", residual=residual)
 
+        q_s = qpe_s = None
         for i in range(cfg.dec_depth):
             d = f"d{i}"
             if i == 0:
                 qkv = ops.gemm(SP(queries), w[d + ".self.qkv.ws"], w[d + ".self.qkv.b"])
                 a = ops.attn_fewkeys(qkv[:, :E], qkv[:, E:2 * E], qkv[:, 2 * E:], B=n, n_heads=Hh, head_dim=32,
-                                     scale=sc32)
-                queries = lin(SP(a), d + ".self.out_proj")
+                                     scale=sc32, split="only")
+                queries = lin(a, d + ".self.out_proj")
             else:
-                qk = ops.gemm(SP(queries, qpe), w[d + ".self.qk.ws"], w[d + ".self.qk.b"])
-                v = lin(SP(queries), d + ".self.v_proj")
-                a = ops.attn_fewkeys(qk[:, :E], qk[:, E:], v, B=n, n_heads=Hh, head_dim=32, scale=sc32)
-                queries = lin(SP(a), d + ".self.out_proj", residual=queries)
+                qk = ops.gemm(qpe_s, w[d + ".self.qk.ws"], w[d + ".self.qk.b"])
+                v = lin(q_s, d + ".self.v_proj")
+                a = ops.attn_fewkeys(qk[:, :E], qk[:, E:], v, B=n, n_heads=Hh, head_dim=32, scale=sc32, split="only")
+                queries = lin(a, d + ".self.out_proj", residual=queries)
             queries = ops.layernorm_rows(queries, w[d + ".norm1.w"], w[d + ".norm1.b"], 1e-5, out_dtype=F32)
             kvq = ops.gemm(SP(keys) if ks is None else ks, w[d + ".kvq.ws"], w[d + ".kvq.b"])
-            queries = ops.layernorm_rows(t2i_attend(d + ".t2i", queries, kvq[:, :Eh], kvq[:, Eh:2 * Eh],
-                                                    w[d + ".t2i.k_pe"], queries),
-                                         w[d + ".norm2.w"], w[d + ".norm2.b"], 1e-5, out_dtype=F32)
-            hmid = lin(SP(queries), d + ".lin1", act="relu")
-            queries = ops.layernorm_rows(lin(SP(hmid), d + ".lin2", residual=queries),
-                                         w[d + ".norm3.w"], w[d + ".norm3.b"], 1e-5, out_dtype=F32)
-            ik = lin(SP(queries, qpe), d + ".i2t.k_proj")
-            iv = lin(SP(queries), d + ".i2t.v_proj")
+            queries, q_s = ln_split(t2i_attend(d + ".t2i", SP(queries, qpe), kvq[:, :Eh], kvq[:, Eh:2 * Eh],
+                                               w[d + ".t2i.k_pe"], queries), d + ".norm2", 1e-5)
+            hmid = lin(q_s, d + ".lin1", act="relu", split="only")
+            queries, q_s = ln_split(lin(hmid, d + ".lin2", residual=queries), d + ".norm3", 1e-5)
+            qpe_s = SP(queries, qpe)
+            ik = lin(qpe_s, d + ".i2t.k_proj")
+            iv = lin(q_s, d + ".i2t.v_proj")
             a = ops.attn_fewkeys(kvq[:, 2 * Eh:], ik, iv, B=n, n_heads=Hh, head_dim=16, scale=sc16, n_q=T,
                                  q_batch_rows=img_rows if shared else None, q_add=w[d + ".i2t.q_pe"])
             last = i + 1 == cfg.dec_depth
@@ -514,21 +522,20 @@
             shared = False
         kvu = ops.gemm(ks, w["dfin.kvu.ws"], w["dfin.kvu.b"])
         kv = kvu[:, :2 * Eh]
-        queries = ops.layernorm_rows(t2i_attend("dfin", queries, kv[:, :Eh], kv[:, Eh:], w["dfin.k_pe"], queries),
-                                     w["dfin.norm.w"], w["dfin.norm.b"], 1e-5, out_dtype=F32)
-        hs = queries.view(n, NT, E)
-
-        def mlp3(prefix: str, x: torch.Tensor) -> torch.Tensor:
-            a = lin(SP(x), prefix + "0", act="relu")
-            a = lin(SP(a), prefix + "1", act="relu")
-            return lin(SP(a), prefix + "2")
+        hs = ops.layernorm_rows(t2i_attend("dfin", qpe_s, kv[:, :Eh], kv[:, Eh:], w["dfin.k_pe"], queries),
+                                w["dfin.norm.w"], w["dfin.norm.b"], 1e-5, split=True).view(n, NT, 3 * E)
+
+        def mlp3(prefix: str, x_split: torch.Tensor) -> torch.Tensor:
+            a = lin(x_split, prefix + "0", act="relu", split="only")
+            a = lin(a, prefix + "1", act="relu", split="only")
+            return lin(a, prefix + "2")
 
         M = n_masks
         if M == 1:
-            hyper = mlp3(_hyp(mask_lo), hs[:, 1 + mask_lo].contiguous()).view(n, 1, 32)
+            hyper = mlp3(_hyp(mask_lo), hs[:, 1 + mask_lo]).view(n, 1, 32)
         else:
-            hyper = torch.stack([mlp3(_hyp(m), hs[:, 1 + m].contiguous()) for m in range(mask_lo, mask_lo + M)], 1)
-        iou = mlp3("iou", hs[:, 0].contiguous())[:, mask_lo:mask_lo + M]
+            hyper = torch.stack([mlp3(_hyp(m), hs[:, 1 + m]) for m in range(mask_lo, mask_lo + M)], 1)
+        iou = mlp3("iou", hs[:, 0])[:, mask_lo:mask_lo + M]
         u0 = kvu[:, 2 * Eh:]
         low = ops.sam_upscale_tail(u0, n, g, w["up1.w"], w["up1.b"], 1e-6, w["up3.blob"], w["up3.b"], hyper)
         return low, iou
```

After: 117.7. About the same (-0.0%).
